# microsoft/M3P

Hardware: AMD Instinct MI355X
Metric: pre-train samples/sec (whole node), 12L/768d seq=128+36 (higher is better)
Workload: dtype bf16; 1 GPU; cfg2: 12L/768d/12h, 36 regions + 128 tokens, V=250002, 19 MLM targets/seq + ITM BCE, dropout 0.10, adam_inverse_sqrt + clip 5; per_gpu_batch=256, global_batch=256, seq_len=164, parallelism=dp1, prewarm_steps=36

## Files before the change

### include/m3p_hip.h

```cpp
#ifndef M3P_HIP_H
#define M3P_HIP_H

#include <stddef.h>
#include <stdint.h>

#ifdef __cplusplus
extern "C" {
#endif

#define M3P_API __attribute__((visibility("default")))

#define M3P_OK 0
#define M3P_EINVAL (-1)
#define M3P_ENOTIMPL (-2)
#define M3P_ENOMEM (-3)

M3P_API const char* m3p_version(void);


enum {
  M3P_EPI_NONE = 0,
  M3P_EPI_BIAS = 1,
  M3P_EPI_BIAS_GELU = 2,
  M3P_EPI_BIAS_DROP_RES = 3,
  M3P_EPI_RES = 4,
  M3P_EPI_DGELU = 5,
  M3P_EPI_MUL = 6,
  M3P_EPI_MULQ = 7,
  M3P_EPI_BIAS_GELUQ = 8,
  M3P_EPI_BIAS_LSE = 9
};

typedef struct M3PEpilogue {
  const float* bias;
  const void* aux;
  void* out2;
  float* colsum;
  int32_t ld_aux;
  int32_t ld_out2;
  int32_t scale_cols;
  float scale;
  float alpha;
  uint32_t seed;
  uint32_t thresh24;
  float inv_keep;
  const float* descale_a;
  const float* descale_b;
  void* out8;
  const float* scale8;
  float* amax8;
  int32_t ld_out8;
  int32_t out8_bf8;
  const int32_t* rng_rows;
  const void* row_ref;
} M3PEpilogue;

M3P_API int m3p_gemm_nt_bf16(const void* A, int lda, const void* W, int ldw, void* C, int ldc,
                             int M, int N, int K, int epilogue, const M3PEpilogue* ep, void* stream);

M3P_API int m3p_gemm_nt_fp8(const void* A8, int lda, int a_is_bf8, const void* W8, int ldw, void* C, int ldc,
                            int M, int N, int K, int epilogue, const M3PEpilogue* ep, void* stream);

M3P_API int m3p_quant_fp8(const void* src, int ld_src, void* dst, int ld_dst, int rows, int cols, const float* scale,
                          float* amax, int bf8, void* stream);

M3P_API int m3p_quant_fp8_batch(const long long* desc, int n_desc, int blocks_per_matrix, void* stream);

M3P_API int m3p_gemm_nt_streamk_f32(const void* A, int lda, const void* W, int ldw, float* C, int ldc,
                                    int M, int N, int K, float alpha, void* stream);
M3P_API int m3p_gemm_nn_streamk_f32(const void* A, int lda, const void* W, int ldw, int k_valid, float* C,
                                    int ldc, int M, int N, int K, float alpha, void* stream);
M3P_API int m3p_gemm_nn_w4_f32(const void* A, int lda, const void* W, int ldw, float* C, int ldc, int M, int N, int K, float alpha,
                               void* workspace, size_t workspace_bytes, void* stream);

M3P_API size_t m3p_gemm_wgrad_workspace_bytes(void);
M3P_API int m3p_gemm_wgrad_bf16(const void* dY, int lddy, const void* X, int ldx, float* dW, int lddw,
                                int M, int N, int K, float alpha, void* workspace, size_t workspace_bytes,
                                void* stream);
M3P_API int m3p_gemm_wgrad_store_bf16(const void* dY, int lddy, const void* X, int ldx, float* dW, int lddw, int M, int N, int K,
                                      float alpha, void* workspace, size_t workspace_bytes, void* stream);
M3P_API int m3p_gemm_wgrad_pair_bf16(const void* dYa, int lddya, const void* Xa, int ldxa, float* dWa, int lddwa, int Na, int Ka,
                                     const void* dYb, int lddyb, const void* Xb, int ldxb, float* dWb, int lddwb, int Nb, int Kb,
                                     int M, float alpha, void* workspace, size_t workspace_bytes, void* stream);


M3P_API int m3p_layernorm_fwd(const void* x, const float* gamma, const float* beta, const uint8_t* rowmask,
                              void* y, float* mean, float* rstd, int rows, int d, float eps, void* stream);

M3P_API int m3p_layernorm_bwd(const void* dy_a, const void* dy_b, const void* x, const float* gamma,
                              const float* mean, const float* rstd, const uint8_t* rowmask,
                              void* dx, void* dx_drop, float* dgamma, float* dbeta, float* dbias_drop,
                              int rows, int d, uint32_t seed, uint32_t thresh24, float inv_keep, void* stream);
M3P_API int m3p_layernorm_bwd_rows(const void* dy_a, const void* dy_b, const void* x, const float* gamma,
                                   const float* mean, const float* rstd, const uint8_t* rowmask,
                                   void* dx, void* dx_drop, float* dgamma, float* dbeta, float* dbias_drop,
                                   int rows, int d, uint32_t seed, uint32_t thresh24, float inv_keep,
                                   const int32_t* rng_rows, void* stream);


M3P_API int m3p_attn_fwd(const void* qkv, const int32_t* keylen, void* ctx, float* lse, uint64_t* keepmask,
                         int B, int S, int H, int dh, uint32_t seed, uint32_t thresh24, float inv_keep,
                         void* stream);

M3P_API int m3p_attn_bwd(const void* qkv, const int32_t* keylen, const void* ctx, const void* dctx,
                         const float* lse, const uint64_t* keepmask, void* dqkv, float* dbias_qkv, int B, int S,
                         int H, int dh, float qscale, uint32_t seed, uint32_t thresh24, float inv_keep,
                         void* stream);

M3P_API int m3p_attn_query_fwd(const void* q, int ld_q, const void* kv, long long kv_bstride, int ld_kv,
                               const int32_t* klen, void* ctx, int B, int Tq, int H, int dh, int Lk, int causal,
                               int pos0, void* stream);

M3P_API int m3p_attn_query_owner_fwd(const void* q, int ld_q, const void* kv, long long kv_bstride, int ld_kv,
                                     const int32_t* klen, void* ctx, int B, int Tq, int H, int dh, int Lk, int causal,
                                     int pos0, const int32_t* owner, int owner_bstride, int owner_kstride, void* stream);

M3P_API int m3p_vocab_select_max_k(void);
M3P_API int m3p_vocab_select_plan(int n, int V, int ld, int beam, int k);
M3P_API size_t m3p_vocab_select_workspace_bytes(int n, int V, int k);
M3P_API int m3p_vocab_select(const void* logits, int ld, int n, int V, const float* beam_scores, int beam, int k,
                             void* workspace, size_t workspace_bytes, float* scores, long long* flat_idx, float* lse,
                             void* stream);

M3P_API int m3p_vocab_sample_plan(int n, int V, int ld, int top_k);
M3P_API size_t m3p_vocab_sample_workspace_bytes(int n, int V, int top_k);
M3P_API int m3p_vocab_sample(const void* logits, int ld, int n, int V, float inv_t, int top_k, uint32_t seed, void* workspace,
                             size_t workspace_bytes, long long* words, float* logprob, float* key, void* stream);

M3P_API int m3p_attn_rows_fwd(const void* q, int ld_q, const void* kv, long long kv_bstride, int ld_kv, const int32_t* klen,
                              void* ctx, float* lse, int B, int Tq, int H, int dh, int Lk, int causal, int pos0,
                              uint32_t seed, uint32_t thresh24, float inv_keep, void* stream);
M3P_API int m3p_attn_rows_bwd(const void* q, int ld_q, const void* kv, long long kv_bstride, int ld_kv, const int32_t* klen,
                              const void* dctx, const float* lse, void* dq, int ld_dq, float* dkv, int B, int Tq, int H,
                              int dh, int Lk, int causal, int pos0, float qscale, uint32_t seed, uint32_t thresh24,
                              float inv_keep, void* stream);

M3P_API int m3p_attn_causal_fwd(const void* qkv, int ld_qkv, void* ctx, float* lse, int B, int T, int H, int dh,
                                uint32_t seed, uint32_t thresh24, float inv_keep, void* stream);
M3P_API int m3p_attn_causal_bwd(const void* qkv, int ld_qkv, const void* dctx, const float* lse, void* dqkv, int ld_dqkv,
                                int B, int T, int H, int dh, float qscale, uint32_t seed, uint32_t thresh24,
                                float inv_keep, void* stream);

M3P_API int m3p_attn_cross_fwd(const void* q, int ld_q, const void* kv, long long kv_bstride, int ld_kv, const int32_t* klen,
                               void* ctx, float* lse, int B, int Tq, int H, int dh, int Lk, uint32_t seed, uint32_t thresh24,
                               float inv_keep, void* stream);
M3P_API int m3p_attn_cross_bwd(const void* q, int ld_q, const void* kv, long long kv_bstride, int ld_kv, const int32_t* klen,
                               const void* dctx, const float* lse, void* dq, int ld_dq, void* dkv, int ld_dkv, int B, int Tq,
                               int H, int dh, int Lk, float qscale, uint32_t seed, uint32_t thresh24, float inv_keep,
                               void* stream);


M3P_API int m3p_cast_f32_bf16(const float* src, void* dst, long long n, void* stream);

M3P_API int m3p_embed_assemble_fwd(const int64_t* tok, const void* emb_bf16, const float* pos,
                                   const void* img_proj, const float* loc, const float* w_loc,
                                   const float* b_loc, const float* g_img, const float* be_img,
                                   const float* g_emb, const float* be_emb, const int32_t* totlen,
                                   void* h, void* z, float* mean_emb, float* rstd_emb, void* e,
                                   float* mean_img, float* rstd_img, int B, int T, int R, int d,
                                   uint32_t seed_img, uint32_t seed_emb, uint32_t thresh24, float inv_keep,
                                   const void* img_rows, void* stream);

M3P_API int m3p_embed_image_rows_fwd(const void* img_proj, const float* loc, const float* w_loc, const float* b_loc,
                                     const float* g_img, const float* be_img, void* e, float* mean_img,
                                     float* rstd_img, void* img_rows, int B, int R, int d, uint32_t seed_img,
                                     uint32_t thresh24, float inv_keep, void* stream);

M3P_API int m3p_embed_assemble_bwd(const void* dh, const void* z, const float* mean_emb, const float* rstd_emb,
                                   const float* g_emb, const void* e, const float* mean_img,
                                   const float* rstd_img, const float* g_img, const int64_t* tok,
                                   const int32_t* totlen, const float* loc, void* dz_scratch, void* de,
                                   float* d_g_emb, float* d_be_emb, float* d_pos, float* d_emb,
                                   void* d_tok_rows, float* d_g_img, float* d_be_img, float* d_b_img, float* d_b_loc,
                                   float* d_w_loc, int B, int T, int R, int d, int pad_index,
                                   uint32_t seed_img, uint32_t seed_emb, uint32_t thresh24, float inv_keep,
                                   int phase, void* stream);


M3P_API int m3p_gather_rows(const void* src, const int32_t* idx, void* dst, int n, int d, void* stream);
M3P_API int m3p_place_rows(const void* src, const int32_t* inv, void* dst, int rows, int d, int n, uint32_t fill_bits,
                           void* stream);
M3P_API int m3p_scatter_add_rows(const void* src, const int32_t* idx, void* dst, int n, int d, void* stream);
M3P_API int m3p_scatter_add_token_rows(const void* rows, int ld_rows, const int64_t* ids, float* dst, int n, int d,
                                       int pad_index, void* stream);

M3P_API int m3p_itm_score_fwd(const void* pre, const float* w2, const float* b2, float* pooled, float* scores, int B,
                              int d, void* stream);
M3P_API int m3p_itm_score_bwd(const float* dscores, const float* pooled, const float* w2, void* dpre16, void* dpreT16,
                              int ldt, float* db1, float* dw2, float* db2, int B, int d, void* stream);

M3P_API int m3p_ce_fwd_bwd(void* logits, int ld, int n_rows, int V, const int64_t* target, float* row_loss,
                           float* loss_sum, float loss_scale, float grad_scale, void* stream);

M3P_API int m3p_ce_lse_from_blocks(const void* stats, int n_blocks, int n_rows, const void* logits, int ld, const int64_t* target,
                                   float* row_loss, float* row_lse, void* scratch, void* stream);
M3P_API int m3p_ce_bwd_colsum(void* logits, int ld, int n_rows, int V, const int64_t* target, const float* row_lse,
                              float grad_scale, float* colsum, void* workspace, size_t workspace_bytes, void* stream);
M3P_API size_t m3p_ce_colsum_workspace_bytes(int ld, int n_rows);
M3P_API int m3p_ce_fwd_bwd_colsum(void* logits, int ld, int n_rows, int V, const int64_t* target, float* row_loss,
                                  float* row_lse, float grad_scale, float* colsum, void* workspace,
                                  size_t workspace_bytes, void* stream);

M3P_API int m3p_ce_shift_target(const void* h, const void* emb, const float* bias, const int64_t* target, float* row_t, void* row_ref,
                                int n_rows, int d, void* stream);
M3P_API int m3p_ce_shift_rows(const void* stats, int n_blocks, int n_rows, float grad_scale, float* row_loss, float* row_s,
                              float* row_q, void* scratch, void* stream);
M3P_API int m3p_ce_shift_colsum(const void* e, int ld, int n_rows, const float* row_s, float* colsum, void* workspace,
                                size_t workspace_bytes, void* stream);
M3P_API int m3p_ce_shift_scale_rows(const void* h, const float* row_s, const float* g, void* out, int n_rows, int d, void* stream);
M3P_API int m3p_ce_shift_target_rows(const void* h, const int64_t* target, const float* row_q, const float* g, float* demb, float* dbias,
                                     int n_rows, int d, void* stream);
M3P_API int m3p_ce_shift_dh(const float* dh32, const void* emb, const int64_t* target, const float* row_s, const float* row_q,
                            const float* g, void* dh, int n_rows, int d, void* stream);

M3P_API int m3p_ce_eval(const void* logits, int ld, int n_rows, int V, const int64_t* target, float* row_loss,
                        int32_t* row_argmax, void* stream);

M3P_API int m3p_colsum_bf16(const void* x, int ld, int n, int ncols, float* out, const float* scale_ptr,
                            void* stream);


M3P_API int m3p_sumsq_f32(const float* g, long long n, double* out, void* stream);

M3P_API int m3p_sumsq_ranges_f32(const float* base, const long long* starts, const long long* counts, int n_ranges, double* out,
                                 void* stream);

M3P_API int m3p_adam_step(float* p, float* g, float* m, float* v, void* w16, long long n, float lr, float beta1,
                          float beta2, float eps, float weight_decay, float step_size, const double* gnorm_sq,
                          float max_norm, float grad_scale, int zero_grad, void* stream);
M3P_API int m3p_adam_step_ranges(float* p, float* g, float* m, float* v, void* w16, const long long* starts,
                                 const long long* counts, const float* step_sizes, const int* zero_grad, int n_ranges,
                                 float lr, float beta1, float beta2, float eps, float weight_decay, const double* gnorm_sq,
                                 float max_norm, float grad_scale, void* stream);

M3P_API int m3p_gelu_fwd(const void* u, void* h, void* dh, long long n, void* stream);
M3P_API int m3p_gelu_fwd_gq(const void* u, void* h, void* gq, int M, int N, void* stream);
M3P_API int m3p_gelu_fwd_q8(const void* u, void* h, void* h8, long long n, const float* scale, float* amax, void* stream);

M3P_API int m3p_gelu_bwd(const void* dy, const void* u, void* du, long long n, void* stream);

M3P_API int m3p_mse_fwd_bwd(const void* pred, int ld_pred, const float* tgt, int ld_tgt, void* dpred, float* row_sq,
                            int rows, int cols, float grad_scale, void* stream);


M3P_API int m3p_dropout_rows(const void* x, int ldx, const void* res, int ldres, void* y, int ldy, int rows, int cols,
                             uint32_t rng_ld, uint32_t rng_col0, uint32_t seed, uint32_t thresh24, float inv_keep,
                             void* stream);

M3P_API int m3p_glu_fwd(const void* ab, int ld_ab, void* y, int rows, int d, void* stream);
M3P_API int m3p_glu_bwd(const void* ab, int ld_ab, const void* dy, void* dab, int rows, int d, void* stream);

M3P_API int m3p_transpose_batch_bf16(const long long* desc, int n_desc, int max_tiles, void* stream);

M3P_API int m3p_transpose_bf16(const void* src, void* dst, int rows, int cols, int ld_src, int ld_dst,
                               void* stream);

M3P_API int m3p_set_persistent_grid(int workgroups);
M3P_API int m3p_set_tile_queue(int32_t* counters, int n_slots);

enum {
  M3P_KERN_NT_SKINNY = 1,
// ... 39 lines not shown
```

### m3p_amd/csrc/attention.hip

```cpp
#include "common.hpp"


namespace {

constexpr int ATTN_BWD_NW = 4;
constexpr int ATTN_BWD_WPS = 3;

static int g_attn_variant = 0;

template <int DH> struct AttnCfg {
  static constexpr int ROWB = DH * 2;
  static constexpr int CH = DH / 8;
  static constexpr int RPI = 1024 / ROWB;
  static constexpr int KK = DH / 32;
  static constexpr int NT = DH / 16;
  static __device__ __forceinline__ int swz(int chunk, int row) { return DH == 64 ? (chunk ^ (row & 7)) : chunk; }
};

__device__ __forceinline__ bf16x4 lds_tr16(const char* p) {
  s16x4 v = __builtin_amdgcn_ds_read_tr16_b64_v4i16((__attribute__((address_space(3))) s16x4*)(p));
  return __builtin_bit_cast(bf16x4, v);
}
__device__ __forceinline__ float row16_sum(float v) {
#define M3P_DPP_ADD(ctrl) v += __builtin_bit_cast(float, __builtin_amdgcn_update_dpp(0, __builtin_bit_cast(int, v), ctrl, 0xf, 0xf, true))
  M3P_DPP_ADD(0xB1);
  M3P_DPP_ADD(0x4E);
  M3P_DPP_ADD(0x124);
  M3P_DPP_ADD(0x128);
#undef M3P_DPP_ADD
  return v;
}
__device__ __forceinline__ uint32_t bit_to_mask(uint32_t bits, int r) {
  uint32_t o;
  switch (r) {
    case 0: asm("v_bfe_i32 %0, %1, 0, 1" : "=v"(o) : "v"(bits)); break;
    case 1: asm("v_bfe_i32 %0, %1, 1, 1" : "=v"(o) : "v"(bits)); break;
    case 2: asm("v_bfe_i32 %0, %1, 2, 1" : "=v"(o) : "v"(bits)); break;
    default: asm("v_bfe_i32 %0, %1, 3, 1" : "=v"(o) : "v"(bits)); break;
  }
  return o;
}
template <int CH>
__device__ __forceinline__ float chunks_sum(float v) {
#define M3P_DPP_ADD(ctrl) v += __builtin_bit_cast(float, __builtin_amdgcn_update_dpp(0, __builtin_bit_cast(int, v), ctrl, 0xf, 0xf, true))
  M3P_DPP_ADD(0xB1);
  M3P_DPP_ADD(0x4E);
  if (CH == 8) M3P_DPP_ADD(0x141);
#undef M3P_DPP_ADD
  return v;
}
__device__ __forceinline__ bf16x8 cat8(bf16x4 a, bf16x4 b) {
  return bf16x8{a[0], a[1], a[2], a[3], b[0], b[1], b[2], b[3]};
}

typedef unsigned int u32x2_t __attribute__((ext_vector_type(2)));
typedef unsigned int u32x4_t __attribute__((ext_vector_type(4)));
template <int NT>
__device__ __forceinline__ void store_row_widened(bf16* row, int fg, bool ok, const bf16x4 (&r)[NT]) {
  static_assert(NT % 2 == 0, "d-tiles are swapped in pairs");
  bf16* p = row + 8 * (fg >> 1) + 16 * (fg & 1);
#pragma unroll
  for (int n0 = 0; n0 < NT; n0 += 2) {
    u32x2_t x = __builtin_bit_cast(u32x2_t, r[n0]), y = __builtin_bit_cast(u32x2_t, r[n0 + 1]);
    asm volatile("s_nop 1\n\tv_permlane16_swap_b32 %0, %2\n\tv_permlane16_swap_b32 %1, %3"
                 : "+v"(x[0]), "+v"(x[1]), "+v"(y[0]), "+v"(y[1]));
    if (ok) *reinterpret_cast<u32x4_t*>(p + 16 * n0) = u32x4_t{x[0], x[1], y[0], y[1]};
  }
}

template <int DH>
__device__ __forceinline__ void stage_rows(const bf16* __restrict__ g, size_t ld, int S, int nrows, char* lds,
                                           int wid, int lane, int nwaves = 4) {
  using Cf = AttnCfg<DH>;
  const int rin = lane / Cf::CH, c = lane % Cf::CH;
  const int ninstr = (nrows + Cf::RPI - 1) / Cf::RPI;
  for (int i = wid; i < ninstr; i += nwaves) {
    const int row = i * Cf::RPI + rin;
    const int gr = min(row, S - 1);
    const int gc = Cf::swz(c, row);
    __builtin_amdgcn_global_load_lds(GLB_PTR(g + (size_t)gr * ld + gc * 8), LDS_PTR(lds + i * 1024), 16, 0, 0);
  }
}

template <int DH>
__device__ __forceinline__ void stage_rows_hidden(const bf16* __restrict__ g, size_t ld, int S, int nrows, char* lds,
                                                  int wid, int lane, int nwaves) {
  using Cf = AttnCfg<DH>;
  const int rin = lane / Cf::CH, c = lane % Cf::CH;
  const int ninstr = (nrows + Cf::RPI - 1) / Cf::RPI;
  const uint32_t lds0 = (uint32_t)(uintptr_t)(__attribute__((address_space(3))) char*)lds;
  for (int i = wid; i < ninstr; i += nwaves) {
    const int row = i * Cf::RPI + rin;
    const int gr = min(row, S - 1);
    const int gc = Cf::swz(c, row);
    const bf16* src = g + (size_t)gr * ld + gc * 8;
    const uint32_t dst = __builtin_amdgcn_readfirstlane(lds0 + (uint32_t)i * 1024u);
    asm volatile("s_mov_b32 m0, %1\n\ts_nop 0\n\tglobal_load_lds_dwordx4 %0, off" :: "v"(src), "s"(dst) : "memory", "m0");
  }
}

template <int DH, int KT, bool DROP, int NTC, int NW = 4, bool EVENS = false>
__global__ __launch_bounds__(NW * 64, NW == 8 ? 2 : 3)
void attn_fwd_kernel(const bf16* __restrict__ qkv, const int* __restrict__ keylen, bf16* __restrict__ ctx,
                     float* __restrict__ lse, unsigned long long* __restrict__ keepmask, int S, int H, int dmodel,
                     uint32_t seed, uint32_t thresh24, float inv_keep) {
  using Cf = AttnCfg<DH>;
  extern __shared__ __attribute__((aligned(16))) char smem[];
  const int tid = threadIdx.x, lane = tid & 63;
  const int wid = __builtin_amdgcn_readfirstlane(tid >> 6);
  const int b = blockIdx.x / H, h = blockIdx.x - b * H;
  const int nt = NTC ? NTC : (S + 15) >> 4;
  const int nk = (nt + 1) >> 1;
  const size_t ld = 3 * (size_t)dmodel;
  const bf16* Qg = qkv + (size_t)b * S * ld + h * DH;
  const bf16* Kg = Qg + dmodel;
  const bf16* Vg = Qg + 2 * dmodel;
  char* sK = smem;
  char* sV = smem + nt * 16 * Cf::ROWB;
  stage_rows<DH>(Kg, ld, S, nt * 16, sK, wid, lane, NW);
  stage_rows<DH>(Vg, ld, S, nk * 32, sV, wid, lane, NW);
  const int fq = lane & 15, fg = lane >> 4;
  const int wrot = (wid + (blockIdx.x >> 3)) & (NW - 1);
  bf16x8 qnext[Cf::KK];
  {
    const int qc0 = min(wrot * 16 + fq, S - 1);
#pragma unroll
    for (int kk = 0; kk < Cf::KK; ++kk)
      qnext[kk] = *reinterpret_cast<const bf16x8*>(Qg + (size_t)qc0 * ld + 32 * kk + 8 * fg);
  }
  const int klen = keylen[b];
  __syncthreads();

  int k_off[Cf::KK];
#pragma unroll
  for (int kk = 0; kk < Cf::KK; ++kk) k_off[kk] = fq * Cf::ROWB + Cf::swz(4 * kk + fg, fq) * 16;
  const int vrow = 4 * fg + (fq >> 2);
  int v_off[Cf::NT];
#pragma unroll
  for (int n = 0; n < Cf::NT; ++n)
    v_off[n] = vrow * Cf::ROWB + Cf::swz(2 * n + ((fq & 3) >> 1), vrow) * 16 + 8 * (fq & 1);

  for (int qb = wrot; qb < nt; qb += NW) {
    const int q = qb * 16 + fq;
    const int qc = min(q, S - 1);
    bf16x8 qf[Cf::KK];
#pragma unroll
    for (int kk = 0; kk < Cf::KK; ++kk) qf[kk] = qnext[kk];
    {
      const int qcn = min(q + 16 * NW, S - 1);
#pragma unroll
      for (int kk = 0; kk < Cf::KK; ++kk)
        qnext[kk] = *reinterpret_cast<const bf16x8*>(Qg + (size_t)qcn * ld + 32 * kk + 8 * fg);
    }

    f32x4 s[2 * KT];
#pragma unroll
    for (int t = 0; t < 2 * KT; ++t) s[t] = f32x4{0.f, 0.f, 0.f, 0.f};
#pragma unroll
    for (int kk = 0; kk < Cf::KK; ++kk) {
#pragma unroll
      for (int t = 0; t < 2 * KT; ++t)
        if (t < nt) {
          const bf16x8 kf = *reinterpret_cast<const bf16x8*>(sK + t * 16 * Cf::ROWB + k_off[kk]);
          s[t] = __builtin_amdgcn_mfma_f32_16x16x32_bf16(kf, qf[kk], s[t], 0, 0, 0);
        }
    }
    constexpr float kLog2e = 1.4426950408889634f;
    float mx = -INFINITY;
    int klen_it = klen;
    asm volatile("" : "+s"(klen_it));
#pragma unroll
    for (int t = 0; t < 2 * KT; ++t)
      if (t < nt) {
        if (16 * t + 16 > klen_it) {
#pragma unroll
          for (int r = 0; r < 4; ++r) s[t][r] = (16 * t + 4 * fg + r < klen_it) ? s[t][r] : -INFINITY;
        }
#pragma unroll
        for (int r = 0; r < 4; ++r) mx = fmaxf(mx, s[t][r]);
      }
    mx = fmaxf(mx, __shfl_xor(mx, 16, 64));
    mx = fmaxf(mx, __shfl_xor(mx, 32, 64));
    const float mx2 = mx * kLog2e;
    float sum = 0.f;
#pragma unroll
    for (int t = 0; t < 2 * KT; ++t)
      if (t < nt) {
#pragma unroll
        for (int r = 0; r < 4; ++r) {
          const float p = __builtin_amdgcn_exp2f(__builtin_fmaf(s[t][r], kLog2e, -mx2));
          s[t][r] = p;
          sum += p;
        }
      }
    sum += __shfl_xor(sum, 16, 64);
    sum += __shfl_xor(sum, 32, 64);
    const float inv = 1.0f / sum;
    const uint32_t rbase = (uint32_t)((b * H + h) * S + qc) * (uint32_t)S;
    const uint32_t thr16 = thresh24 >> 8;
    const bool even_rows = EVENS || (S & 1) == 0;
    unsigned long long* mrow = keepmask ? keepmask + ((size_t)(b * H + h) * nt + qb) * nt * 4 : nullptr;
    constexpr int MW = (8 * KT + 63) / 64;
    uint32_t mlo[MW], mhi[MW];
#pragma unroll
    for (int g = 0; g < MW; ++g) mlo[g] = mhi[g] = 0u;
    bf16x8 pf[KT];
#pragma unroll
    for (int kk = 0; kk < KT; ++kk) {
      float p[8];
      const float invk = DROP ? inv * inv_keep : inv;
      bool kq[8] = {true, true, true, true, true, true, true, true};
      if (DROP) {
#pragma unroll
        for (int hf = 0; hf < 2; ++hf) {
          const int t = 2 * kk + hf;
          if (t < nt) {
            const uint32_t base = rbase + (uint32_t)(16 * t + 4 * fg);
            bool k4[4];
            if (even_rows) {
              asm volatile("" ::: "memory");
              const uint32_t h0 = m3p_hash32(base >> 1, seed), h1 = m3p_hash32((base >> 1) + 1u, seed);
              k4[0] = (h0 & 0xFFFFu) >= thr16; k4[1] = (h0 >> 16) >= thr16;
              k4[2] = (h1 & 0xFFFFu) >= thr16; k4[3] = (h1 >> 16) >= thr16;
            } else {
              asm volatile("" ::: "memory");
              m3p_keep_run<4>(base, seed, thresh24, k4);
            }
#pragma unroll
            for (int r = 0; r < 4; ++r) kq[4 * hf + r] = k4[r];
          }
        }
      }
#pragma unroll
      for (int hf = 0; hf < 2; ++hf) {
        const int t = 2 * kk + hf;
        unsigned long long kw[4] = {0ull, 0ull, 0ull, 0ull};
#pragma unroll
        for (int r = 0; r < 4; ++r) {
          const int j = 4 * hf + r;
          float v = 0.f;
          if (t < nt) {
            v = s[t][r] * invk;
            if (DROP) {
              const bool keep = kq[j];
              kw[r] = __builtin_amdgcn_ballot_w64(keep);
              v = keep ? v : 0.f;
            }
          }
          p[j] = v;
        }
        if (DROP && t < nt) {
          asm("s_nop 3\n\tv_writelane_b32 %0, %2, %10\n\tv_writelane_b32 %1, %3, %10\n\tv_writelane_b32 %0, %4, %11\n\tv_writelane_b32 %1, %5, %11\n\t"
              "v_writelane_b32 %0, %6, %12\n\tv_writelane_b32 %1, %7, %12\n\tv_writelane_b32 %0, %8, %13\n\tv_writelane_b32 %1, %9, %13"
              : "+v"(mlo[(4 * t) >> 6]), "+v"(mhi[(4 * t) >> 6])
              : "s"((uint32_t)kw[0]), "s"((uint32_t)(kw[0] >> 32)), "s"((uint32_t)kw[1]), "s"((uint32_t)(kw[1] >> 32)),
                "s"((uint32_t)kw[2]), "s"((uint32_t)(kw[2] >> 32)), "s"((uint32_t)kw[3]), "s"((uint32_t)(kw[3] >> 32)),
                "i"((4 * t) & 63), "i"((4 * t + 1) & 63), "i"((4 * t + 2) & 63), "i"((4 * t + 3) & 63));
        }
      }
      pf[kk] = bf16x8{(bf16)p[0], (bf16)p[1], (bf16)p[2], (bf16)p[3], (bf16)p[4], (bf16)p[5], (bf16)p[6], (bf16)p[7]};
    }
    if (DROP && mrow) {
#pragma unroll
      for (int g = 0; g < MW; ++g)
        if (64 * g + lane < 4 * nt) mrow[64 * g + lane] = ((unsigned long long)mhi[g] << 32) | mlo[g];
    }
    f32x4 o[Cf::NT];
#pragma unroll
    for (int n = 0; n < Cf::NT; ++n) o[n] = f32x4{0.f, 0.f, 0.f, 0.f};
#pragma unroll
    for (int kk = 0; kk < KT; ++kk) {
      if (kk < nk) {
#pragma unroll
        for (int n = 0; n < Cf::NT; ++n) {
          const char* pv = sV + kk * 32 * Cf::ROWB + v_off[n];
          const bf16x8 vf = cat8(lds_tr16(pv), lds_tr16(pv + 16 * Cf::ROWB));
          o[n] = __builtin_amdgcn_mfma_f32_16x16x32_bf16(vf, pf[kk], o[n], 0, 0, 0);
        }
      }
    }
    {
      bf16x4 ob[Cf::NT];
#pragma unroll
      for (int n = 0; n < Cf::NT; ++n) ob[n] = bf16x4{(bf16)o[n][0], (bf16)o[n][1], (bf16)o[n][2], (bf16)o[n][3]};
      store_row_widened<Cf::NT>(ctx + (size_t)(b * S + min(q, S - 1)) * dmodel + h * DH, fg, q < S, ob);
      if (q < S && fg == 0) lse[(size_t)(b * H + h) * S + q] = mx + __logf(sum);
    }
  }
}

template <int DH, int KT, bool DROP, bool MASK, int NKC, int NTC, int NW = 4, int KB = 1, int KBQ = KB, bool ONEPASS = false>
__global__ __launch_bounds__(NW * 64, NTC == 11 ? ATTN_BWD_WPS : ((NW == 8 || KB == 2) ? 2 : 3))
void attn_bwd_kernel(const bf16* __restrict__ qkv, const int* __restrict__ keylen, const bf16* __restrict__ ctx,
                     const bf16* __restrict__ dctx, const float* __restrict__ lse,
                     const unsigned long long* __restrict__ keepmask, bf16* __restrict__ dqkv,
                     float* __restrict__ dbias_qkv, int S, int H, int dmodel, float qscale, uint32_t seed,
                     uint32_t thresh24, float inv_keep) {
  using Cf = AttnCfg<DH>;
  extern __shared__ __attribute__((aligned(16))) char smem[];
  const int tid = threadIdx.x, lane = tid & 63;
  const int wid = __builtin_amdgcn_readfirstlane(tid >> 6);
  const int b = blockIdx.x / H, h = blockIdx.x - b * H;
  const int wrot = (NW & (NW - 1)) ? wid : ((wid + (blockIdx.x >> 3)) & (NW - 1));
  const int nt = NTC ? NTC : ((S + 15) >> 4);
  const int nk = NKC ? NKC : ((S + 31) >> 5);
  const size_t ld = 3 * (size_t)dmodel;
  const int b_rd = b;
  const bf16* Qg = qkv + (size_t)b_rd * S * ld + h * DH;
  const bf16* Kg = Qg + dmodel;
  const bf16* Vg = Qg + 2 * dmodel;
  const bf16* Og = ctx + (size_t)b_rd * S * dmodel + h * DH;
  const bf16* dOg = dctx + (size_t)b_rd * S * dmodel + h * DH;
  bf16* dQg = dqkv + (size_t)b * S * ld + h * DH;
  bf16* dKg = dQg + dmodel;
  bf16* dVg = dQg + 2 * dmodel;
  const float* lse_bh = lse + (size_t)(b * H + h) * S;
  const int klen = keylen[b];
  const unsigned long long* mbh = MASK ? keepmask + (size_t)(b * H + h) * nt * nt * 4 : nullptr;

  const int tile_bytes = nk * 32 * Cf::ROWB;
  char* s0 = smem;
  char* s1 = smem + tile_bytes;
  float* sL = reinterpret_cast<float*>(smem + 2 * tile_bytes);
  float* sD = sL + nk * 32;
  const int fq = lane & 15, fg = lane >> 4;
  float* sB = sD + nk * 32;
  float* sBw = sB + wid * 3 * DH;
  constexpr int DSP = NTC * 32;
  char* sK = reinterpret_cast<char*>(sB + NW * 3 * DH);
  char* sDS = sK + tile_bytes;
  static_assert(!ONEPASS || (NKC == 6 && NTC == 11 && KB == 1 && DH == 64), "ONEPASS is the M3P-sequence instantiation");
  f32x4 bsum[Cf::NT];
#pragma unroll
  for (int n = 0; n < Cf::NT; ++n) bsum[n] = f32x4{0.f, 0.f, 0.f, 0.f};
  auto bias_acc = [&](int, int n, const bf16x4& v4) {
    bsum[n] += f32x4{(float)v4[0], (float)v4[1], (float)v4[2], (float)v4[3]};
  };
  auto bias_flush = [&](int part) {
#pragma unroll
    for (int n = 0; n < Cf::NT; ++n) {
      f32x4 x = bsum[n];
#pragma unroll
      for (int r = 0; r < 4; ++r) x[r] = row16_sum(x[r]);
      if (fq == 0) *reinterpret_cast<f32x4*>(sBw + part * DH + 16 * n + 4 * fg) = x;
      bsum[n] = f32x4{0.f, 0.f, 0.f, 0.f};
    }
  };

  int r_off[Cf::KK];
#pragma unroll
  for (int kk = 0; kk < Cf::KK; ++kk) r_off[kk] = fq * Cf::ROWB + Cf::swz(4 * kk + fg, fq) * 16;
  const int trow = 4 * fg + (fq >> 2);
  int t_off[Cf::NT];
#pragma unroll
  for (int n = 0; n < Cf::NT; ++n)
    t_off[n] = trow * Cf::ROWB + Cf::swz(2 * n + ((fq & 3) >> 1), trow) * 16 + 8 * (fq & 1);

#define PAD_TILE(t) (NTC ? (t) >= NTC : (!MASK && (t) >= nt))
  constexpr float kLog2e = 1.4426950408889634f;
  constexpr float kMasked = -1.0e30f;
  constexpr bool kDfromLds = NKC != 0;
  constexpr int kStageInstr = NKC * 32 / Cf::RPI;
  constexpr int kNIW = kDfromLds ? (kStageInstr + NW - 1) / NW : 1;
  bf16x8 orow[kNIW];
  if (kDfromLds) {
    const int rin = lane / Cf::CH, c = lane % Cf::CH;
#pragma unroll
    for (int j = 0; j < kNIW; ++j) {
      const int row = (wid + j * NW) * Cf::RPI + rin;
      orow[j] = *reinterpret_cast<const bf16x8*>(Og + (size_t)min(row, S - 1) * dmodel + Cf::swz(c, row) * 8);
    }
  }
  stage_rows<DH>(Qg, ld, S, nk * 32, s0, wid, lane, NW);
  stage_rows<DH>(dOg, (size_t)dmodel, S, nk * 32, s1, wid, lane, NW);
  if (ONEPASS) stage_rows<DH>(Kg, ld, S, nk * 32, sK, wid, lane, NW);
  bf16x8 kf[KB][Cf::KK], vf[KB][Cf::KK];
  auto load_kv = [&](int u, int kb) {
    const int keyc = min(kb * 16 + fq, S - 1);
#pragma unroll
    for (int kk = 0; kk < Cf::KK; ++kk) {
      kf[u][kk] = *reinterpret_cast<const bf16x8*>(Kg + (size_t)keyc * ld + 32 * kk + 8 * fg);
      vf[u][kk] = *reinterpret_cast<const bf16x8*>(Vg + (size_t)keyc * ld + 32 * kk + 8 * fg);
    }
  };
  constexpr bool kNextFrag = NKC != 0 && NTC != 0 && !(DROP && !MASK);
  bf16x8 kfn[KB][Cf::KK], vfn[KB][Cf::KK];
  auto load_kv_next = [&](int u, int kb) {
    const int keyc = min(kb * 16 + fq, S - 1);
#pragma unroll
    for (int kk = 0; kk < Cf::KK; ++kk) {
      kfn[u][kk] = *reinterpret_cast<const bf16x8*>(Kg + (size_t)keyc * ld + 32 * kk + 8 * fg);
      vfn[u][kk] = *reinterpret_cast<const bf16x8*>(Vg + (size_t)keyc * ld + 32 * kk + 8 * fg);
    }
  };
  if (wrot * KB < nt) {
#pragma unroll
    for (int u = 0; u < KB; ++u) load_kv(u, wrot * KB + u);
  }
  const float log2_inv_keep = DROP ? __builtin_amdgcn_logf(inv_keep) : 0.f;
  const float keep_prob = DROP ? __builtin_amdgcn_rcpf(inv_keep) : 1.f;
  for (int q = tid; q < nk * 32; q += NW * 64) {
    float dsum = 0.f, l = INFINITY;
    if (q < S) {
      if (!kDfromLds) {
        const bf16* op = Og + (size_t)q * dmodel;
        const bf16* dp = dOg + (size_t)q * dmodel;
#pragma unroll
        for (int c = 0; c < DH / 8; ++c) {
          const bf16x8 ov = *reinterpret_cast<const bf16x8*>(op + 8 * c);
          const bf16x8 dv = *reinterpret_cast<const bf16x8*>(dp + 8 * c);
#pragma unroll
          for (int e = 0; e < 8; ++e) dsum += (float)ov[e] * (float)dv[e];
        }
      }
      l = lse_bh[q] * kLog2e - log2_inv_keep;
    }
    if (!kDfromLds) sD[q] = dsum * keep_prob;
    sL[q] = l;
  }
  if (kDfromLds) {
    asm volatile("s_waitcnt vmcnt(0)" ::: "memory");
    const int rin = lane / Cf::CH, c = lane % Cf::CH;
#pragma unroll
    for (int j = 0; j < kNIW; ++j) {
      const int i = wid + j * NW;
      if (i < kStageInstr) {
        const bf16x8 dv = *reinterpret_cast<const bf16x8*>(s1 + i * 1024 + lane * 16);
        float part = 0.f;
#pragma unroll
        for (int e = 0; e < 8; ++e) part += (float)orow[j][e] * (float)dv[e];
        part = chunks_sum<Cf::CH>(part);
        const int row = i * Cf::RPI + rin;
        if (c == 0) sD[row] = row < S ? part * keep_prob : 0.f;
      }
    }
  }
  __syncthreads();

  constexpr bool kPreA = MASK && NKC != 0;
// ... 209 lines not shown
  }
  __syncthreads();

  for (int qb0 = wrot * KBQ; qb0 < nt; qb0 += NW * KBQ) {
    int q[KBQ], qc[KBQ];
    float lq[KBQ], dq_[KBQ];
    uint32_t rbase[KBQ];
#pragma unroll
    for (int u = 0; u < KBQ; ++u) {
      q[u] = (qb0 + u) * 16 + fq;
      qc[u] = min(q[u], S - 1);
      if (kNextFrag) {
        if (qb0 != wrot * KBQ) {
#pragma unroll
          for (int kk = 0; kk < Cf::KK; ++kk) { qf[u][kk] = qfn[u][kk]; df[u][kk] = dfn[u][kk]; }
        }
        if (qb0 + NW * KBQ < nt) load_qd_next(u, qb0 + NW * KBQ + u);
      } else if (qb0 != wrot * KBQ) {
        load_qd(u, qb0 + u);
      }
      const bool in = q[u] < nk * 32;
      lq[u] = in ? sL[min(q[u], nk * 32 - 1)] : INFINITY;
      dq_[u] = in ? sD[min(q[u], nk * 32 - 1)] : 0.f;
      rbase[u] = (uint32_t)((b * H + h) * S + qc[u]) * (uint32_t)S;
    }
    int klen_it = klen;
    asm volatile("" : "+s"(klen_it));
    constexpr bool kPreB = MASK && NKC != 0;
    unsigned long long mwB[2][KBQ][2][4];
    auto mask_words_B = [&](int kq_, int par) {
#pragma unroll
      for (int u = 0; u < KBQ; ++u)
#pragma unroll
        for (int hf = 0; hf < 2; ++hf) {
          const unsigned long long* mw_ = mbh + ((size_t)min(qb0 + u, nt - 1) * nt + min(2 * kq_ + hf, nt - 1)) * 4;
#pragma unroll
          for (int r = 0; r < 4; ++r) mwB[par][u][hf][r] = mw_[r];
        }
    };
    if (kPreB) mask_words_B(0, 0);
    f32x4 dq[KBQ][Cf::NT];
#pragma unroll
    for (int u = 0; u < KBQ; ++u)
#pragma unroll
      for (int n = 0; n < Cf::NT; ++n) dq[u][n] = f32x4{0.f, 0.f, 0.f, 0.f};
#pragma unroll(NKC ? NKC : 1)
    for (int kq = 0; kq < nk; ++kq) {
      if (kPreB && kq + 1 < nk) mask_words_B(kq + 1, (kq + 1) & 1);
      f32x4 scB[KBQ][2], dpB[KBQ][2];
#pragma unroll
      for (int u = 0; u < KBQ; ++u)
#pragma unroll
        for (int hf = 0; hf < 2; ++hf) {
          scB[u][hf] = f32x4{0.f, 0.f, 0.f, 0.f};
          dpB[u][hf] = DROP ? f32x4{0.f, 0.f, 0.f, 0.f} : f32x4{-dq_[u], -dq_[u], -dq_[u], -dq_[u]};
        }
#pragma unroll
      for (int kk = 0; kk < Cf::KK; ++kk) {
#pragma unroll
        for (int hf = 0; hf < 2; ++hf) {
          const int t = 2 * kq + hf;
          if (PAD_TILE(t)) continue;
          const bf16x8 kfr = *reinterpret_cast<const bf16x8*>(s0 + t * 16 * Cf::ROWB + r_off[kk]);
          const bf16x8 vfr = *reinterpret_cast<const bf16x8*>(s1 + t * 16 * Cf::ROWB + r_off[kk]);
#pragma unroll
          for (int u = 0; u < KBQ; ++u) {
            scB[u][hf] = __builtin_amdgcn_mfma_f32_16x16x32_bf16(kfr, qf[u][kk], scB[u][hf], 0, 0, 0);
            dpB[u][hf] = __builtin_amdgcn_mfma_f32_16x16x32_bf16(vfr, df[u][kk], dpB[u][hf], 0, 0, 0);
          }
        }
      }
      bf16x8 sfrag[KBQ];
#pragma unroll
      for (int u = 0; u < KBQ; ++u) {
        f32x4 ds2[2];
#pragma unroll
        for (int hf = 0; hf < 2; ++hf) {
          const int t = 2 * kq + hf;
          if (PAD_TILE(t)) {
            ds2[hf] = f32x4{0.f, 0.f, 0.f, 0.f};
            continue;
          }
          f32x4 sc = scB[u][hf];
          const f32x4 dp = dpB[u][hf];
          const unsigned long long* mw = MASK ? mbh + ((size_t)min(qb0 + u, nt - 1) * nt + min(t, nt - 1)) * 4 : nullptr;
          if (16 * t + 16 > klen_it) {
            asm volatile("");
#pragma unroll
            for (int r = 0; r < 4; ++r) sc[r] = (16 * t + 4 * fg + r < klen_it) ? sc[r] : kMasked;
          }
#pragma unroll
          for (int r = 0; r < 4; ++r) {
            const int key = 16 * t + 4 * fg + r;
            const float p = __builtin_amdgcn_exp2f(__builtin_fmaf(sc[r], kLog2e, -lq[u]));
            if (DROP) {
              float kfac;
              if (MASK) {
                asm("v_cndmask_b32_e64 %0, 0, 1.0, %1" : "=v"(kfac) : "s"(kPreB ? mwB[kq & 1][u][hf][r] : mw[r]));
              } else {
                static_assert(MASK || !DROP, "dropout in backward reads the forward pass's keep words");
                kfac = 1.f;
              }
              ds2[hf][r] = p * __builtin_fmaf(dp[r], kfac, -dq_[u]);
            } else {
              ds2[hf][r] = p * dp[r];
            }
          }
        }
        sfrag[u] = bf16x8{(bf16)ds2[0][0], (bf16)ds2[0][1], (bf16)ds2[0][2], (bf16)ds2[0][3],
                          (bf16)ds2[1][0], (bf16)ds2[1][1], (bf16)ds2[1][2], (bf16)ds2[1][3]};
      }
#pragma unroll
      for (int n = 0; n < Cf::NT; ++n) {
        const char* pk = s0 + kq * 32 * Cf::ROWB + t_off[n];
        const bf16x8 kT = cat8(lds_tr16(pk), lds_tr16(pk + 16 * Cf::ROWB));
#pragma unroll
        for (int u = 0; u < KBQ; ++u) dq[u][n] = __builtin_amdgcn_mfma_f32_16x16x32_bf16(kT, sfrag[u], dq[u][n], 0, 0, 0);
      }
      if (NKC) __builtin_amdgcn_sched_barrier(0);
    }
#pragma unroll
    for (int u = 0; u < KBQ; ++u) {
      bf16x4 qb4[Cf::NT];
#pragma unroll
      for (int n = 0; n < Cf::NT; ++n)
        qb4[n] = bf16x4{(bf16)(dq[u][n][0] * qscale), (bf16)(dq[u][n][1] * qscale), (bf16)(dq[u][n][2] * qscale), (bf16)(dq[u][n][3] * qscale)};
      const bool ok = q[u] < S;
      if (dbias_qkv) {
#pragma unroll
        for (int n = 0; n < Cf::NT; ++n) bias_acc(0, n, ok ? qb4[n] : bf16x4{0, 0, 0, 0});
      }
      store_row_widened<Cf::NT>(dQg + (size_t)qc[u] * ld, fg, ok, qb4);
    }
  }
  }

  if (dbias_qkv) {
    bias_flush(0);
    __syncthreads();
    for (int i = tid; i < 3 * DH; i += NW * 64) {
      const int part = i / DH, c = i - part * DH;
      if (part != 1) {
        float tot = 0.f;
#pragma unroll
        for (int w = 0; w < NW; ++w) tot += sB[w * 3 * DH + i];
        atomicAdd(dbias_qkv + part * dmodel + h * DH + c, tot);
      }
    }
  }
}

#undef PAD_TILE

template <bool DROP, bool MASK>
__global__ __launch_bounds__(768, 3)
void attn_bwd_p_kernel(const bf16* __restrict__ qkv, const int* __restrict__ keylen, const bf16* __restrict__ ctx,
                       const bf16* __restrict__ dctx, const float* __restrict__ lse,
                       const unsigned long long* __restrict__ keepmask, bf16* __restrict__ dqkv,
                       float* __restrict__ dbias_qkv, int S, int H, int dmodel, int nheads, float qscale, float inv_keep) {
  constexpr int DH = 64, NW = 12, NKC = 6, NTC = 11, NR = NKC * 32;
  using Cf = AttnCfg<DH>;
  constexpr int DSP = NTC * 32;
  constexpr int TILE = NR * Cf::ROWB;
  extern __shared__ __attribute__((aligned(16))) char smem[];
  const int tid = threadIdx.x, lane = tid & 63;
  const int wid = __builtin_amdgcn_readfirstlane(tid >> 6);
  char* s0 = smem;
  char* s1 = s0 + TILE;
  char* sK = s1 + TILE;
  char* sDS = sK + TILE;
  float* sL = reinterpret_cast<float*>(sDS + NTC * 16 * DSP);
  float* sD = sL + NR;
  float* sB = sD + NR;
  unsigned long long* sMW = reinterpret_cast<unsigned long long*>(sB + 2 * NW * 3 * DH) + wid * 48;
  const size_t ld = 3 * (size_t)dmodel;
  const int fq = lane & 15, fg = lane >> 4;
  const int rin = lane / Cf::CH, c8 = lane % Cf::CH;
  int r_off[Cf::KK];
#pragma unroll
  for (int kk = 0; kk < Cf::KK; ++kk) r_off[kk] = fq * Cf::ROWB + Cf::swz(4 * kk + fg, fq) * 16;
  const int trow = 4 * fg + (fq >> 2);
  int t_off[Cf::NT];
#pragma unroll
  for (int n = 0; n < Cf::NT; ++n)
    t_off[n] = trow * Cf::ROWB + Cf::swz(2 * n + ((fq & 3) >> 1), trow) * 16 + 8 * (fq & 1);
  constexpr float kLog2e = 1.4426950408889634f;
  constexpr float kMasked = -1.0e30f;
  const float log2_inv_keep = DROP ? __builtin_amdgcn_logf(inv_keep) : 0.f;
  const float keep_prob = DROP ? __builtin_amdgcn_rcpf(inv_keep) : 1.f;
  constexpr int kStageInstr = NR / Cf::RPI;
  constexpr int kNIW = (kStageInstr + NW - 1) / NW;
#define PAD_TILE(t) ((t) >= NTC)

  bf16x8 orow[kNIW], kf[Cf::KK], vf[Cf::KK];
  float lse_r = 0.f;
  unsigned long long mw_req = 0;
  auto request_head = [&](int hd) {
    const int b = hd / H, h = hd - b * H;
    const bf16* Qg = qkv + (size_t)b * S * ld + h * DH;
    const bf16* Og = ctx + (size_t)b * S * dmodel + h * DH;
    const bf16* dOg = dctx + (size_t)b * S * dmodel + h * DH;
#pragma unroll
    for (int j = 0; j < kNIW; ++j) {
      const int row = (wid + j * NW) * Cf::RPI + rin;
      orow[j] = *reinterpret_cast<const bf16x8*>(Og + (size_t)min(row, S - 1) * dmodel + Cf::swz(c8, row) * 8);
    }
    stage_rows_hidden<DH>(Qg, ld, S, NR, s0, wid, lane, NW);
    stage_rows_hidden<DH>(dOg, (size_t)dmodel, S, NR, s1, wid, lane, NW);
    const int keyc = min(min(wid, NTC - 1) * 16 + fq, S - 1);
#pragma unroll
    for (int kk = 0; kk < Cf::KK; ++kk) {
      kf[kk] = *reinterpret_cast<const bf16x8*>(Qg + dmodel + (size_t)keyc * ld + 32 * kk + 8 * fg);
      vf[kk] = *reinterpret_cast<const bf16x8*>(Qg + 2 * dmodel + (size_t)keyc * ld + 32 * kk + 8 * fg);
    }
    if (tid < NR && tid < S) lse_r = lse[(size_t)hd * S + tid];
    if (MASK && lane < 4 * NTC)
      mw_req = keepmask[(size_t)hd * NTC * NTC * 4 + ((size_t)(lane >> 2) * NTC + min(wid, NTC - 1)) * 4 + (lane & 3)];
  };

  f32x4 bsum[Cf::NT];
#pragma unroll
  for (int n = 0; n < Cf::NT; ++n) bsum[n] = f32x4{0.f, 0.f, 0.f, 0.f};
  auto bias_acc = [&](int n, const bf16x4& v4) { bsum[n] += f32x4{(float)v4[0], (float)v4[1], (float)v4[2], (float)v4[3]}; };
  auto bias_flush = [&](float* slot, int part) {
    float t[2][4], u[4];
#pragma unroll
    for (int n = 0; n < 2; ++n)
#pragma unroll
      for (int r = 0; r < 4; ++r) {
        asm volatile("v_add_f32_dpp %0, %1, %1 row_ror:8 row_mask:0xf bank_mask:0x3" : "=v"(t[n][r]) : "v"(bsum[n][r]));
        asm volatile("v_add_f32_dpp %0, %1, %1 row_ror:8 row_mask:0xf bank_mask:0xc" : "+v"(t[n][r]) : "v"(bsum[n + 2][r]));
      }
    asm volatile("s_nop 1");
#pragma unroll
    for (int r = 0; r < 4; ++r) {
      asm volatile("v_add_f32_dpp %0, %1, %1 row_half_mirror row_mask:0xf bank_mask:0x5" : "=v"(u[r]) : "v"(t[0][r]));
      asm volatile("v_add_f32_dpp %0, %1, %1 row_half_mirror row_mask:0xf bank_mask:0xa" : "+v"(u[r]) : "v"(t[1][r]));
    }
    asm volatile("s_nop 1");
    f32x4 x;
#pragma unroll
    for (int r = 0; r < 4; ++r) {
      float v = u[r];
      v += __builtin_bit_cast(float, __builtin_amdgcn_update_dpp(0, __builtin_bit_cast(int, v), 0xB1, 0xf, 0xf, true));
      v += __builtin_bit_cast(float, __builtin_amdgcn_update_dpp(0, __builtin_bit_cast(int, v), 0x4E, 0xf, 0xf, true));
      x[r] = v;
    }
    if ((fq & 3) == 0) *reinterpret_cast<f32x4*>(slot + part * DH + 16 * (fq >> 2) + 4 * fg) = x;
#pragma unroll
    for (int n = 0; n < Cf::NT; ++n) bsum[n] = f32x4{0.f, 0.f, 0.f, 0.f};
  };
  auto bias_reduce = [&](const float* slots, int h) {
    for (int i = tid; i < 3 * DH; i += NW * 64) {
      const int part = i / DH, c = i - part * DH;
      if (part != 1) {
        float tot = 0.f;
#pragma unroll
        for (int w = 0; w < NW; ++w) tot += slots[w * 3 * DH + i];
        atomicAdd(dbias_qkv + part * dmodel + h * DH + c, tot);
      }
    }
  };

  bf16x4 kb4[Cf::NT], vb4[Cf::NT], qb4[Cf::NT];
  const int key = wid * 16 + fq;
  bf16* dQg_prev = nullptr;
  auto store_head = [&](bf16* dQh) {
    if (wid < NTC) {
      bf16* row = dQh + (size_t)min(key, S - 1) * ld;
      store_row_widened<Cf::NT>(row, fg, key < S, qb4);
      store_row_widened<Cf::NT>(row + dmodel, fg, key < S, kb4);
      store_row_widened<Cf::NT>(row + 2 * dmodel, fg, key < S, vb4);
    }
  };
  int hd = blockIdx.x;
  if (hd >= nheads) return;
  constexpr int kStagger = 2;
  for (int i = 0; i < (int)((blockIdx.x >> 3) & 3) * kStagger; ++i) __builtin_amdgcn_s_sleep(16);
  request_head(hd);
  int par = 0, prev_h = -1;
  for (;;) {
    const int b = hd / H, h = hd - b * H;
    bf16* dQg = dqkv + (size_t)b * S * ld + h * DH;
    const bf16* Kg = qkv + (size_t)b * S * ld + h * DH + dmodel;
    const int klen = keylen[b];
    float* sBh = sB + par * (NW * 3 * DH);
    __builtin_amdgcn_s_waitcnt(0x0F70);
    asm volatile("s_waitcnt vmcnt(0)" ::: "memory");
#pragma unroll
    for (int j = 0; j < kNIW; ++j) {
      const int i = wid + j * NW;
      if (i < kStageInstr) {
        const bf16x8 dvv = *reinterpret_cast<const bf16x8*>(s1 + i * 1024 + lane * 16);
        float part = 0.f;
#pragma unroll
        for (int e = 0; e < 8; ++e) part += (float)orow[j][e] * (float)dvv[e];
        part = chunks_sum<Cf::CH>(part);
        const int row = i * Cf::RPI + rin;
        if (c8 == 0) sD[row] = row < S ? part * keep_prob : 0.f;
      }
    }
    if (tid < NR) sL[tid] = tid < S ? lse_r * kLog2e - log2_inv_keep : INFINITY;
    if (MASK && lane < 4 * NTC) sMW[lane] = mw_req;
    asm volatile("s_waitcnt lgkmcnt(0)" ::: "memory");
    __builtin_amdgcn_s_barrier();
    asm volatile("" ::: "memory");
    if (prev_h >= 0 && dbias_qkv) bias_reduce(sB + (par ^ 1) * (NW * 3 * DH), prev_h);
    if (prev_h >= 0) store_head(dQg_prev);
    dQg_prev = dQg;
    stage_rows_hidden<DH>(Kg, ld, S, NR, sK, wid, lane, NW);
    if (wid < NTC) {
      const float kbias = (key < klen) ? 0.f : kMasked;
      f32x4 dv[Cf::NT], dk[Cf::NT];
#pragma unroll
      for (int n = 0; n < Cf::NT; ++n) dv[n] = dk[n] = f32x4{0.f, 0.f, 0.f, 0.f};
#pragma unroll
      for (int kq = 0; kq < NKC; ++kq) {
        f32x4 scA[2], dpA[2], dnegA[2];
#pragma unroll
        for (int hf = 0; hf < 2; ++hf) {
          const int t = 2 * kq + hf;
          dnegA[hf] = f32x4{-sD[16 * t + 4 * fg + 0], -sD[16 * t + 4 * fg + 1], -sD[16 * t + 4 * fg + 2], -sD[16 * t + 4 * fg + 3]};
          scA[hf] = f32x4{kbias, kbias, kbias, kbias};
          dpA[hf] = DROP ? f32x4{0.f, 0.f, 0.f, 0.f} : dnegA[hf];
        }
#pragma unroll
        for (int kk = 0; kk < Cf::KK; ++kk) {
#pragma unroll
          for (int hf = 0; hf < 2; ++hf) {
            const int t = 2 * kq + hf;
            if (PAD_TILE(t)) continue;
            const bf16x8 qf = *reinterpret_cast<const bf16x8*>(s0 + t * 16 * Cf::ROWB + r_off[kk]);
            const bf16x8 df = *reinterpret_cast<const bf16x8*>(s1 + t * 16 * Cf::ROWB + r_off[kk]);
            scA[hf] = __builtin_amdgcn_mfma_f32_16x16x32_bf16(qf, kf[kk], scA[hf], 0, 0, 0);
            dpA[hf] = __builtin_amdgcn_mfma_f32_16x16x32_bf16(df, vf[kk], dpA[hf], 0, 0, 0);
          }
        }
        f32x4 pd2[2], ds2[2];
#pragma unroll
        for (int hf = 0; hf < 2; ++hf) {
          const int t = 2 * kq + hf;
          if (PAD_TILE(t)) {
            pd2[hf] = ds2[hf] = f32x4{0.f, 0.f, 0.f, 0.f};
            continue;
          }
          uint32_t kbits = 0;
          if (MASK) kbits = (uint32_t)(sMW[4 * t + (fq & 3)] >> (4 * fg + 16 * (fq >> 2)));
#pragma unroll
          for (int r = 0; r < 4; ++r) {
            const int q = 16 * t + 4 * fg + r;
            const float p = __builtin_amdgcn_exp2f(__builtin_fmaf(scA[hf][r], kLog2e, -sL[q]));
            if (DROP) {
              const float pd = __builtin_bit_cast(float, __builtin_bit_cast(uint32_t, p) & bit_to_mask(kbits, r));
              pd2[hf][r] = pd;
              ds2[hf][r] = __builtin_fmaf(pd, dpA[hf][r], p * dnegA[hf][r]);
            } else {
              pd2[hf][r] = p;
              ds2[hf][r] = p * dpA[hf][r];
            }
          }
        }
        const bf16x8 pfrag = bf16x8{(bf16)pd2[0][0], (bf16)pd2[0][1], (bf16)pd2[0][2], (bf16)pd2[0][3],
                                    (bf16)pd2[1][0], (bf16)pd2[1][1], (bf16)pd2[1][2], (bf16)pd2[1][3]};
        const bf16x8 sfrag = bf16x8{(bf16)ds2[0][0], (bf16)ds2[0][1], (bf16)ds2[0][2], (bf16)ds2[0][3],
                                    (bf16)ds2[1][0], (bf16)ds2[1][1], (bf16)ds2[1][2], (bf16)ds2[1][3]};
#pragma unroll
        for (int hf = 0; hf < 2; ++hf) {
          if (PAD_TILE(2 * kq + hf)) continue;
          *reinterpret_cast<bf16x4*>(sDS + key * DSP + (32 * kq + 16 * hf + 4 * fg) * 2) =
              hf ? bf16x4{sfrag[4], sfrag[5], sfrag[6], sfrag[7]} : bf16x4{sfrag[0], sfrag[1], sfrag[2], sfrag[3]};
        }
#pragma unroll
        for (int n = 0; n < Cf::NT; ++n) {
          const char* pq = s0 + kq * 32 * Cf::ROWB + t_off[n];
          const char* pdo = s1 + kq * 32 * Cf::ROWB + t_off[n];
          const bf16x8 qT = cat8(lds_tr16(pq), lds_tr16(pq + 16 * Cf::ROWB));
          const bf16x8 dT = cat8(lds_tr16(pdo), lds_tr16(pdo + 16 * Cf::ROWB));
          dv[n] = __builtin_amdgcn_mfma_f32_16x16x32_bf16(dT, pfrag, dv[n], 0, 0, 0);
          dk[n] = __builtin_amdgcn_mfma_f32_16x16x32_bf16(qT, sfrag, dk[n], 0, 0, 0);
        }
        __builtin_amdgcn_sched_barrier(0);
      }
#pragma unroll
      for (int n = 0; n < Cf::NT; ++n) {
        kb4[n] = bf16x4{(bf16)dk[n][0], (bf16)dk[n][1], (bf16)dk[n][2], (bf16)dk[n][3]};
        vb4[n] = bf16x4{(bf16)dv[n][0], (bf16)dv[n][1], (bf16)dv[n][2], (bf16)dv[n][3]};
        if (dbias_qkv) bias_acc(n, key < S ? vb4[n] : bf16x4{0, 0, 0, 0});
      }
    }
    if (dbias_qkv) bias_flush(sBh + wid * 3 * DH, 2);
    __builtin_amdgcn_s_waitcnt(0);
    asm volatile("s_waitcnt vmcnt(0) lgkmcnt(0)" ::: "memory");
    __builtin_amdgcn_s_barrier();
    asm volatile("" ::: "memory");
    const int next = hd + gridDim.x;
    if (next < nheads) request_head(next);
    if (wid < NTC) {
      f32x4 dq[Cf::NT];
#pragma unroll
      for (int n = 0; n < Cf::NT; ++n) dq[n] = f32x4{0.f, 0.f, 0.f, 0.f};
      const char* pds = sDS + trow * DSP + wid * 32 + (fq & 3) * 8;
#pragma unroll
      for (int kq = 0; kq < NKC; ++kq) {
        const bf16x4 lo = lds_tr16(pds + (32 * kq) * DSP);
        const bf16x4 hi = PAD_TILE(2 * kq + 1) ? bf16x4{0, 0, 0, 0} : lds_tr16(pds + (32 * kq + 16) * DSP);
        const bf16x8 sfr = cat8(lo, hi);
#pragma unroll
        for (int n = 0; n < Cf::NT; ++n) {
          const char* pk = sK + kq * 32 * Cf::ROWB + t_off[n];
          const bf16x8 kT = cat8(lds_tr16(pk), lds_tr16(pk + 16 * Cf::ROWB));
          dq[n] = __builtin_amdgcn_mfma_f32_16x16x32_bf16(kT, sfr, dq[n], 0, 0, 0);
        }
      }
#pragma unroll
      for (int n = 0; n < Cf::NT; ++n) {
        qb4[n] = bf16x4{(bf16)(dq[n][0] * qscale), (bf16)(dq[n][1] * qscale), (bf16)(dq[n][2] * qscale), (bf16)(dq[n][3] * qscale)};
        if (dbias_qkv) bias_acc(n, key < S ? qb4[n] : bf16x4{0, 0, 0, 0});
      }
    }
    if (dbias_qkv) bias_flush(sBh + wid * 3 * DH, 0);
    prev_h = h;
    par ^= 1;
    if (next >= nheads) break;
    hd = next;
  }
  store_head(dQg_prev);
  if (dbias_qkv) {
    __syncthreads();
    bias_reduce(sB + (par ^ 1) * (NW * 3 * DH), prev_h);
  }
#undef PAD_TILE
}

template <int DH>
int launch_fwd(const bf16* qkv, const int* keylen, bf16* ctx, float* lse, unsigned long long* keepmask, int B, int S, int H,
               int dmodel, uint32_t seed, uint32_t thresh24, float inv_keep, hipStream_t st) {
  const int nt = (S + 15) / 16, nk = (S + 31) / 32;
  const size_t lds = (size_t)(nt * 16 + nk * 32) * DH * 2;
  const bool wide = 2 * lds > 160 * 1024;
#define M3P_ATTN_FWD(KT)                                                                                        \
  do {                                                                                                          \
    constexpr int NW0 = (KT == 16) ? 8 : 4;    \
    auto kern = thresh24 ? attn_fwd_kernel<DH, KT, true, 0, NW0> : attn_fwd_kernel<DH, KT, false, 0, NW0>;       \
    if (nt == 11 && KT == 6) kern = thresh24 ? ((S & 1) ? attn_fwd_kernel<DH, 6, true, 11> : attn_fwd_kernel<DH, 6, true, 11, 4, true>) \
                                             : attn_fwd_kernel<DH, 6, false, 11>; \
    if (wide) kern = thresh24 ? attn_fwd_kernel<DH, KT, true, 0, 8> : attn_fwd_kernel<DH, KT, false, 0, 8>;       \
    hipError_t e = hipFuncSetAttribute((const void*)kern, hipFuncAttributeMaxDynamicSharedMemorySize, (int)lds); \
    if (e != hipSuccess) return (int)e;                                                                         \
    hipLaunchKernelGGL(kern, dim3(B* H), dim3((wide || NW0 == 8) ? 512 : 256), lds, st, qkv, keylen, ctx, lse, keepmask, S, H, dmodel, seed, \
                       thresh24, inv_keep);                                                                     \
  } while (0)
  if (nk <= 6) M3P_ATTN_FWD(6);
  else if (nk <= 12) M3P_ATTN_FWD(12);
  else if (nk <= 16) M3P_ATTN_FWD(16);
  else return M3P_EINVAL;
#undef M3P_ATTN_FWD
  M3P_CHECK_LAUNCH();
  return M3P_OK;
}

template <int DH>
int launch_bwd(const bf16* qkv, const int* keylen, const bf16* ctx, const bf16* dctx, const float* lse,
               const unsigned long long* keepmask, bf16* dqkv, float* dbias, int B, int S, int H, int dmodel, float qscale,
               uint32_t seed, uint32_t thresh24, float inv_keep, hipStream_t st) {
  const int nk = (S + 31) / 32;
  const bool wide = (size_t)2 * ((size_t)2 * nk * 32 * DH * 2) > 160 * 1024;
  const bool m3p_seq = nk == 6 && (S + 15) / 16 == 11;
  const bool onepass = m3p_seq && DH == 64 && (!thresh24 || keepmask) && !(g_attn_variant & 1);
  const int nwaves = wide ? 8 : (onepass ? 12 : (m3p_seq ? ATTN_BWD_NW : 4));
  const size_t lds = (size_t)2 * nk * 32 * DH * 2 + (size_t)2 * nk * 32 * sizeof(float) + 3 * nwaves * DH * sizeof(float) +
                     (onepass ? (size_t)nk * 32 * DH * 2 + (size_t)11 * 16 * 11 * 32 : 0);
#define M3P_ATTN_BWD(KT, DROP, MASK)                                                                            \
  do {                                                                                                          \
    auto kern = attn_bwd_kernel<DH, KT, DROP, MASK, 0, 0>;                                                      \
    if (wide) kern = attn_bwd_kernel<DH, KT, DROP, MASK, 0, 0, 8>;                                              \
    if (nk == 6) kern = attn_bwd_kernel<DH, KT, DROP, MASK, 6, 0>;                                              \
    if (m3p_seq) kern = attn_bwd_kernel<DH, KT, DROP, MASK, 6, 11, ATTN_BWD_NW, 1, 1>;                                \
    if constexpr (DH == 64 && (MASK || !DROP)) { if (onepass) kern = attn_bwd_kernel<DH, KT, DROP, MASK, 6, 11, 12, 1, 1, true>; } \
    hipError_t e = hipFuncSetAttribute((const void*)kern, hipFuncAttributeMaxDynamicSharedMemorySize, (int)lds); \
    if (e != hipSuccess) return (int)e;                                                                         \
    hipLaunchKernelGGL(kern, dim3(B* H), dim3(nwaves * 64), lds, st, qkv, keylen, ctx, dctx, lse, keepmask, dqkv, dbias, S, H, \
                       dmodel, qscale, seed, thresh24, inv_keep);                                               \
  } while (0)
  if (nk > 16) return M3P_EINVAL;
  if constexpr (DH == 64) {
    if (onepass && !(g_attn_variant & 2)) {
      int dev = 0, n_cu = 0;
      if (hipGetDevice(&dev) != hipSuccess || hipDeviceGetAttribute(&n_cu, hipDeviceAttributeMultiprocessorCount, dev) != hipSuccess || n_cu <= 0)
        n_cu = 256;
      const size_t ldsp = (size_t)3 * 192 * 128 + (size_t)11 * 16 * 11 * 32 + 2 * 192 * sizeof(float) + 2 * 12 * 3 * 64 * sizeof(float) + 12 * 48 * 8;
      auto kp = thresh24 ? attn_bwd_p_kernel<true, true> : attn_bwd_p_kernel<false, false>;
      if (hipFuncSetAttribute((const void*)kp, hipFuncAttributeMaxDynamicSharedMemorySize, (int)ldsp) == hipSuccess) {
        const int nheads = B * H;
        hipLaunchKernelGGL(kp, dim3(nheads < n_cu ? nheads : n_cu), dim3(768), ldsp, st, qkv, keylen, ctx, dctx, lse, keepmask, dqkv, dbias,
                           S, H, dmodel, nheads, qscale, inv_keep);
        M3P_CHECK_LAUNCH();
        return M3P_OK;
      }
      (void)hipGetLastError();
    }
  }
  if (!thresh24) M3P_ATTN_BWD(16, false, false);
  else M3P_ATTN_BWD(16, true, true);
#undef M3P_ATTN_BWD
  M3P_CHECK_LAUNCH();
  return M3P_OK;
}

}

extern "C" {

void m3p_debug_attn_variant(int v) { g_attn_variant = v; }

int m3p_attn_fwd(const void* qkv, const int32_t* keylen, void* ctx, float* lse, uint64_t* keepmask, int B, int S, int H, int dh,
                 uint32_t seed, uint32_t thresh24, float inv_keep, void* stream) {
  if (B <= 0 || S <= 0 || H <= 0 || S > 512) return M3P_EINVAL;
  if (((uintptr_t)qkv & 15) || ((uintptr_t)ctx & 7)) return M3P_EINVAL;
  const int dmodel = H * dh;
  hipStream_t st = (hipStream_t)stream;
  if (dh == 64) return launch_fwd<64>((const bf16*)qkv, keylen, (bf16*)ctx, lse, (unsigned long long*)keepmask, B, S, H, dmodel, seed, thresh24, inv_keep, st);
  if (dh == 32) return launch_fwd<32>((const bf16*)qkv, keylen, (bf16*)ctx, lse, (unsigned long long*)keepmask, B, S, H, dmodel, seed, thresh24, inv_keep, st);
  return M3P_EINVAL;
}

int m3p_attn_bwd(const void* qkv, const int32_t* keylen, const void* ctx, const void* dctx, const float* lse,
                 const uint64_t* keepmask, void* dqkv, float* dbias_qkv, int B, int S, int H, int dh, float qscale,
                 uint32_t seed, uint32_t thresh24, float inv_keep, void* stream) {
  if (B <= 0 || S <= 0 || H <= 0 || S > 512) return M3P_EINVAL;
  if (thresh24 && !keepmask) return M3P_EINVAL;
  if (((uintptr_t)qkv & 15) || ((uintptr_t)ctx & 15) || ((uintptr_t)dctx & 15) || ((uintptr_t)dqkv & 7)) return M3P_EINVAL;
  const int dmodel = H * dh;
  hipStream_t st = (hipStream_t)stream;
  if (dh == 64)
    return launch_bwd<64>((const bf16*)qkv, keylen, (const bf16*)ctx, (const bf16*)dctx, lse, (const unsigned long long*)keepmask, (bf16*)dqkv, dbias_qkv, B, S, H,
                          dmodel, qscale, seed, thresh24, inv_keep, st);
  if (dh == 32)
    return launch_bwd<32>((const bf16*)qkv, keylen, (const bf16*)ctx, (const bf16*)dctx, lse, (const unsigned long long*)keepmask, (bf16*)dqkv, dbias_qkv, B, S, H,
                          dmodel, qscale, seed, thresh24, inv_keep, st);
  return M3P_EINVAL;
}

}
```

### m3p_amd/functional.py

```python
import math
import os
from collections import OrderedDict

import torch

from . import lib as L
from . import fp8 as fp8mod
from . import ops
from . import rng

BF16 = torch.bfloat16
ALIGN = 64
BUCKET_ALIGN = 64 * 8


def _round_up(n, a):
    return (n + a - 1) // a * a


_VOCAB_FULL_TILES = os.environ.get('M3P_VOCAB_FULL_TILES', '1') != '0'
_GELU_GRAD_IN_FWD = os.environ.get('M3P_GELU_GRAD_IN_FWD', '0') != '0'
_GELU_BYTE_GRAD = int(os.environ.get('M3P_GELU_BYTE_GRAD', '2'))
_CE_FUSED_LSE = os.environ.get('M3P_CE_FUSED_LSE', '1') != '0'
_VOCAB_DGRAD_W4 = os.environ.get('M3P_VOCAB_DGRAD_W4', '1') != '0'
# ... 257 lines not shown
        self.out = [ar.w('encoder_attn.%d.out_lin.weight' % i) for i in range(n)]
        self.bq = [ar.xattn(i, 'bq') for i in range(n)]
        self.bkv = [ar.xattn(i, 'bkv') for i in range(n)]
        self.bo = [ar.p('encoder_attn.%d.out_lin.bias' % i) for i in range(n)]


_REF_SITE0 = 1 << 20


def _transposed(w):
    wt = torch.empty((w.shape[1], w.shape[0]), dtype=BF16, device=w.device)
    ops.transpose_bf16(w, wt)
    return wt


def refiner_fwd(model, x, keylen, B, R, seed_step, p):
    ar = model.arena()
    d, H = model.dim, model.n_heads
    dh = d // H
    M = B * R
    qscale = 1.0 / math.sqrt(dh)
    seed = lambda i, k: rng.stream_seed(model.base_seed, seed_step, _REF_SITE0 + 8 * i + k)
    layers = []
    for i in range(model.n_refine_layers):
        pre = 'refine_embeddings.layers.%d.' % i
        xn, mean_a, rstd_a = ops.layernorm_fwd(x, ar.p(pre + 'sublayer.0.norm.weight'), ar.p(pre + 'sublayer.0.norm.bias'))
        qkv = ops.gemm_nt(xn, ar.ref_qkv_w16(i), L.EPI_BIAS, bias=ar.ref_qkv_bias(i), scale_cols=d, scale=qscale)
        ctxt, lse, kmask = ops.attn_fwd(qkv, keylen, B, R, H, dh, seed=seed(i, 0), p_drop=p, want_mask=True)
        cat = torch.empty((M, 2 * d), dtype=BF16, device=x.device)
        ops.dropout_rows(ctxt, p, seed(i, 1), out=cat[:, :d], rng_ld=2 * d, rng_col0=0)
        ops.dropout_rows(xn, p, seed(i, 1), out=cat[:, d:], rng_ld=2 * d, rng_col0=d)
        ab = ops.gemm_nt(cat, ar.w(pre + 'self_attn.aoa_layer.0.weight'), L.EPI_BIAS,
                         bias=ar.p(pre + 'self_attn.aoa_layer.0.bias'))
        x1 = ops.dropout_rows(ops.glu_fwd(ab), p, seed(i, 2), res=x)
        xn2, mean_b, rstd_b = ops.layernorm_fwd(x1, ar.p(pre + 'sublayer.1.norm.weight'), ar.p(pre + 'sublayer.1.norm.bias'))
        u = torch.empty((M, 4 * d), dtype=BF16, device=x.device)
        hact = ops.gemm_nt(xn2, ar.w(pre + 'feed_forward.lin1.weight'), L.EPI_BIAS_GELU,
                           bias=ar.p(pre + 'feed_forward.lin1.bias'), out2=u)
        t = ops.gemm_nt(hact, ar.w(pre + 'feed_forward.lin2.weight'), L.EPI_BIAS, bias=ar.p(pre + 'feed_forward.lin2.bias'))
        if p > 0:
            ops.dropout_rows(t, p, seed(i, 3), out=t)
        x2 = ops.dropout_rows(t, p, seed(i, 4), res=x1)
        layers.append((x, mean_a, rstd_a, xn, qkv, ctxt, lse, kmask, cat, ab, x1, mean_b, rstd_b, xn2, u, hact))
        x = x2
    out, mean_f, rstd_f = ops.layernorm_fwd(x, ar.p('refine_embeddings.norm.weight'), ar.p('refine_embeddings.norm.bias'))
    return out, (layers, x, mean_f, rstd_f)


def refiner_bwd(model, dout, saved, keylen, B, R, seed_step, p):
    ar = model.arena()
    d, H = model.dim, model.n_heads
    dh = d // H
    seed = lambda i, k: rng.stream_seed(model.base_seed, seed_step, _REF_SITE0 + 8 * i + k)
    layers, x_last, mean_f, rstd_f = saved
    dx, _ = ops.layernorm_bwd(dout, None, x_last, ar.p('refine_embeddings.norm.weight'), mean_f, rstd_f, None,
                              ar.g('refine_embeddings.norm.weight'), ar.g('refine_embeddings.norm.bias'))
    for i in reversed(range(model.n_refine_layers)):
        pre = 'refine_embeddings.layers.%d.' % i
        (x, mean_a, rstd_a, xn, qkv, ctxt, lse, kmask, cat, ab, x1, mean_b, rstd_b, xn2, u, hact) = layers[i]
        layers[i] = None
        dt = ops.dropout_rows(dx, p, seed(i, 4))
        if p > 0:
            ops.dropout_rows(dt, p, seed(i, 3), out=dt)
        ops.colsum(dt, d, ar.g(pre + 'feed_forward.lin2.bias'))
        ops.gemm_wgrad(dt, hact, ar.g(pre + 'feed_forward.lin2.weight'))
        du = ops.gemm_nt(dt, _transposed(ar.w(pre + 'feed_forward.lin2.weight')), L.EPI_DGELU, aux=u,
                         colsum=ar.g(pre + 'feed_forward.lin1.bias'))
        ops.gemm_wgrad(du, xn2, ar.g(pre + 'feed_forward.lin1.weight'))
        dxn2 = ops.gemm_nt(du, _transposed(ar.w(pre + 'feed_forward.lin1.weight')), L.EPI_NONE)
        dln, _ = ops.layernorm_bwd(dxn2, None, x1, ar.p(pre + 'sublayer.1.norm.weight'), mean_b, rstd_b, None,
                                   ar.g(pre + 'sublayer.1.norm.weight'), ar.g(pre + 'sublayer.1.norm.bias'))
        dx1 = ops.dropout_rows(dln, 0.0, 0, res=dx)
        del dt, du, dxn2, dln, u, hact, xn2
        dy = ops.dropout_rows(dx1, p, seed(i, 2))
        dab = ops.glu_bwd(ab, dy)
        ops.colsum(dab, 2 * d, ar.g(pre + 'self_attn.aoa_layer.0.bias'))
        ops.gemm_wgrad(dab, cat, ar.g(pre + 'self_attn.aoa_layer.0.weight'))
        dcat = ops.gemm_nt(dab, _transposed(ar.w(pre + 'self_attn.aoa_layer.0.weight')), L.EPI_NONE)
        dctx = ops.dropout_rows(dcat[:, :d], p, seed(i, 1), rng_ld=2 * d, rng_col0=0)
        dxn_cat = ops.dropout_rows(dcat[:, d:], p, seed(i, 1), rng_ld=2 * d, rng_col0=d)
        dqkv = ops.attn_bwd(qkv, keylen, ctxt, dctx, lse, B, R, H, dh, dbias_qkv=ar.ref_qkv_bias(i, grad=True),
                            seed=seed(i, 0), p_drop=p, keepmask=kmask)
        ops.gemm_wgrad(dqkv, xn, ar.ref_qkv_wgrad(i))
        dxn = ops.gemm_nt(dqkv, _transposed(ar.ref_qkv_w16(i)), L.EPI_RES, aux=dxn_cat)
        dln, _ = ops.layernorm_bwd(dxn, None, x, ar.p(pre + 'sublayer.0.norm.weight'), mean_a, rstd_a, None,
                                   ar.g(pre + 'sublayer.0.norm.weight'), ar.g(pre + 'sublayer.0.norm.bias'))
        dx = ops.dropout_rows(dln, 0.0, 0, res=dx1)
        del dy, dab, dcat, dctx, dxn_cat, dqkv, dxn, dln, dx1
    ar.touch(*[n for n in ar.names if n.startswith('refine_embeddings.')])
    return dx


class GradSink:

    def __init__(self):
        self.buf = None

    def rows(self, like):
        if self.buf is None:
            self.buf = torch.zeros_like(like)
        assert self.buf.shape == like.shape
        return self.buf

    def take(self):
        buf, self.buf = self.buf, None
        return buf


def _sink_of(tensor, base):
    root = tensor._base if tensor._is_view() else tensor
    sink = getattr(root, '_m3p_sink', None) if root is not None else None
    if sink is None or base is None or not torch.is_grad_enabled():
        return None
    if root.dim() != 2 or not root.is_contiguous() or root.storage_offset() != 0 or tuple(root.shape) != tuple(base.shape):
        return None
    return sink


def first_rows_sink(model, tensor):
    d = model.dim
    if tensor.dim() != 3 or tensor.dtype != BF16 or not tensor._is_view():
        return None, None, None
    st, soff = tensor.stride(), tensor.storage_offset()
    if st[2] != 1 or st[0] % d or soff % d:
        return None, None, None
    with torch.no_grad():
        base = torch.as_strided(tensor, (tensor.untyped_storage().nbytes() // 2 // d, d), (d, 1), 0)
    sink = _sink_of(tensor, base)
    if sink is None:
        return None, None, None
    cache = model.__dict__.setdefault('_first_rows_cache', {})
    key = (tensor.shape[0], st[0], soff, tensor.device)
    rows = cache.get(key)
    if rows is None:
        rows = ((soff + torch.arange(tensor.shape[0], device=tensor.device, dtype=torch.int64) * st[0]) // d).to(torch.int32)
        cache.clear()
        cache[key] = rows
    return sink, base, rows


N_ENC_ARGS = 17

ROW_TILE = 256
COMPACT_MIN_ROWS = 4096


def compact_rows_eligible(n_rows, M):
    if n_rows <= 0:
        return 0
    n = _round_up(n_rows, ROW_TILE)
    return n if (n >= COMPACT_MIN_ROWS and 2 * n <= M) else 0


class OutputRows:

    def __init__(self, flags):
        flags = torch.as_tensor(flags).reshape(-1).cpu()
        if flags.dtype != torch.bool:
            flags = flags != 0
        self.flags = flags
        self.M = int(flags.numel())
        sel = torch.nonzero(flags).view(-1)
        self.n_rows = int(sel.numel())
        self.n = compact_rows_eligible(self.n_rows, self.M)
        self.idx = self.idx64 = self.inv = None
        if self.n:
            pad = torch.nonzero(~flags).view(-1)[:self.n - self.n_rows]
            idx = torch.cat([sel, pad]).to(torch.int32)
            inv = torch.full((self.M,), -1, dtype=torch.int32)
            inv[sel] = torch.arange(self.n_rows, dtype=torch.int32)
            self._host = (idx, inv)

    @classmethod
    def from_masks(cls, B, S, R, first=True, pred_mask=None, region_labels=None):
        flags = torch.zeros((B, S), dtype=torch.bool)
        if first:
            flags[:, 0] = True
        if pred_mask is not None:
            flags[:, R:] |= torch.as_tensor(pred_mask).cpu().reshape(S - R, B).t() != 0
        if region_labels is not None and R > 0:
            flags[:, :R] |= torch.as_tensor(region_labels).cpu().reshape(B, R) != -1
        return cls(flags)

    def to(self, device):
        if self.n and self.idx is None:
            from .utils import to_cuda
            with torch.cuda.device(device):
                self.idx, self.inv = to_cuda(*self._host)
            self.idx64 = self.idx.long()
        assert self.idx is None or self.idx.device == torch.device(device), 'an OutputRows serves one pass on one device'
        return self


class EncoderFn(torch.autograd.Function):

    @staticmethod
    def forward(ctx, anchor, model, x, lengths, x_img, lengths_img, image_loc, p_drop, p_attn, seed_step, p_refine=None,
                track=False, text_embed=None, langs=None, h0=None, positions=None, out_rows=None):
        ar = model.arena()
        ready = model.ddp_hook.params_ready if model.ddp_hook is not None else (lambda key: None)
        ar.refresh(wait_params=False)
        ready('vocab')
        ready('embed')
        dev = ar.device
        d, H, nL = model.dim, model.n_heads, model.n_layers
        dh = d // H
        seed = lambda kind, i=0: rng.stream_seed(model.base_seed, seed_step, _site(kind, i))
        if h0 is not None:
            assert x is None and x_img is None and text_embed is None and langs is None and positions is None
            B = lengths.shape[0]
            S = h0.shape[0] // B
            T, R, M = S, 0, B * S
            totlen, rowmask = ops.seq_masks(lengths.to(device=dev, dtype=torch.int64).contiguous(), None, B, S)
            h = h0.detach().to(BF16).contiguous()
            ximg16 = loc = emb_saved = img_rows = img_saved = ref_saved = keylen_img = tok = None
        else:
            h = None
            T, B = x.shape
            R = 0 if x_img is None else x_img.shape[0]
            S = R + T
            M = B * S
            x = x.to(dev).contiguous()
        if h is None:
            table, tok = ar.w('embeddings.weight'), x
            if text_embed is not None:
                assert tuple(text_embed.shape) == (B, T, d), (tuple(text_embed.shape), (B, T, d))
                table = text_embed.detach().to(device=dev, dtype=BF16).contiguous().view(B * T, d)
                tok = (torch.arange(B, device=dev, dtype=torch.int64) * T)[None, :] + \
                    torch.arange(T, device=dev, dtype=torch.int64)[:, None]
                tok = tok.contiguous()
            if langs is not None or positions is not None:
                assert text_embed is None and R == 0
                rows = table[x.t()].float()
                if langs is not None:
                    langs = langs.to(dev).contiguous()
                    rows = rows + ar.p('cross_lang_embeddings.weight')[langs.t()]
                if positions is not None:
                    positions = positions.to(dev).contiguous()
                    assert positions.size() == (T, B)
                    ptab = ar.p('position_embeddings.weight')
                    rows = rows + ptab[positions.t()] - ptab[:T][None, :, :]
                table = rows.to(BF16).reshape(B * T, d).contiguous()
                tok = ((torch.arange(B, device=dev, dtype=torch.int64) * T)[None, :] +
                       torch.arange(T, device=dev, dtype=torch.int64)[:, None]).contiguous()
            totlen, rowmask = ops.seq_masks(lengths.to(device=dev, dtype=torch.int64).contiguous(),
                                            None if R == 0 else lengths_img.to(device=dev, dtype=torch.int64).contiguous(), B, S)

            ximg16 = img_proj = loc = None
            if R > 0:
                xi = x_img.detach().to(dev)
                if xi.dtype == torch.float32 and xi.stride(2) == 1 and xi.stride(0) % 4 == 0 and xi.stride(1) % 4 == 0:
                    ximg16 = ops.cast_rows_bf16(xi)
                else:
                    ximg16 = ops.cast_bf16(xi.contiguous().view(R * B, 2048))
                loc = image_loc.contiguous().float()
                img_proj = ops.gemm_nt(ximg16, ar.w('image_embeddings.image_embeddings.weight'), L.EPI_BIAS,
                                       bias=ar.p('image_embeddings.image_embeddings.bias'))
            img_rows = img_saved = ref_saved = keylen_img = None
            if p_refine is not None and R > 0:
                rows, img_saved = ops.embed_image_rows_fwd(
                    img_proj, loc, ar.p('image_embeddings.image_location_embeddings.weight'),
                    ar.p('image_embeddings.image_location_embeddings.bias'), ar.p('image_embeddings.LayerNorm.weight'),
                    ar.p('image_embeddings.LayerNorm.bias'), B, R, d, seed_img=seed('img'), p_drop=p_drop)
                keylen_img = lengths_img.to(device=dev, dtype=torch.int32).contiguous()
                img_rows, ref_saved = refiner_fwd(model, rows, keylen_img, B, R, seed_step, p_refine)
            h, emb_saved = ops.embed_assemble_fwd(
                tok, table, ar.p('position_embeddings.weight'), img_proj, loc,
                ar.p('image_embeddings.image_location_embeddings.weight'),
                ar.p('image_embeddings.image_location_embeddings.bias'),
                ar.p('image_embeddings.LayerNorm.weight'), ar.p('image_embeddings.LayerNorm.bias'),
                ar.p('layer_norm_emb.weight'), ar.p('layer_norm_emb.bias'), totlen, B, T, R, d,
                seed_img=seed('img'), seed_emb=seed('emb'), p_drop=p_drop, img_rows=img_rows, img_saved=img_saved)

        saved_layers = []
        qscale = 1.0 / math.sqrt(dh)
        st8 = model.fp8_state() if model.fp8 else None
        if st8 is not None:
            assert M % 256 == 0, 'the fp8 GEMM takes whole 256-row tiles (B * S %% 256 == 0): M = %d' % M
            if model.training:
                st8.roll()
            ready(None)
            st8.quant_weights(ar)

        def lin(xin, i, xsite, wsite, w16, epi, pre8=None, **kw):
            if st8 is None or wsite not in fp8mod.FWD_SITES:
                return ops.gemm_nt(xin, w16, epi, **kw)
            x8, dxs = pre8 if pre8 is not None else st8.quant(xin, i, xsite)
            w8, _, dws = st8.weights[(i, wsite)]
            return ops.gemm_nt_fp8(x8, w8, epi, descale_a=dxs, descale_b=dws, **kw)

        rows_c = None
        if out_rows is not None and out_rows.n and track and st8 is None and nL > 0 and d % 8 == 0 \
                and ops.gq_eligible(M, 4 * d) == ops.gq_eligible(out_rows.n, 4 * d):
            assert out_rows.M == M, 'out_rows was built for %d rows, this pass has %d' % (out_rows.M, M)
            rows_c = out_rows.to(dev)

        for i in range(nL):
            a, f = 'attentions.%d.' % i, 'ffns.%d.' % i
            ready(('layer', i))
            qkv = lin(h, i, 'x', 'wqkv', ar.qkv_w16(i), L.EPI_BIAS, bias=ar.qkv_bias(i), scale_cols=d, scale=qscale)
            ctxt, lse, kmask = ops.attn_fwd(qkv, totlen, B, S, H, dh, seed=seed('attn_p', i), p_drop=p_attn,
                                            want_mask=True)
            lse = (lse, kmask)
            compact = rows_c is not None and i == nL - 1
            Mi, ctx_in, res_in, mask_i, rr, ctx_c = M, ctxt, h, rowmask, {}, None
            if compact:
                Mi, rr = rows_c.n, dict(rng_rows=rows_c.idx)
                ctx_in = ctx_c = ops.gather_rows(ctxt, rows_c.idx, Mi, d)
                res_in = ops.gather_rows(h, rows_c.idx, Mi, d)
                mask_i = rowmask[rows_c.idx64]
            pre1 = lin(ctx_in, i, 'ctx', 'wout', ar.w(a + 'out_lin.weight'), L.EPI_BIAS_DROP_RES, bias=ar.p(a + 'out_lin.bias'),
                       aux=res_in, seed=seed('attn_out', i), p_drop=p_drop, **rr)
            x1, mean1, rstd1 = ops.layernorm_fwd(pre1, ar.p('layer_norm1.%d.weight' % i), ar.p('layer_norm1.%d.bias' % i))
            hact8 = None
            u_holds_grad = False
            if (st8 is None or 'w1' not in fp8mod.FWD_SITES) and not _GELU_GRAD_IN_FWD and _GELU_BYTE_GRAD == 2 and track \
                    and ops.gq_eligible(Mi, 4 * d):
                u = torch.empty((Mi * 4 * d,), dtype=torch.uint8, device=dev)
                o8 = {}
                if st8 is not None and 'w2' in fp8mod.FWD_SITES:
                    kh = st8.index(i, 'hact')
                    if st8.seen[kh]:
                        o8 = dict(out8=torch.empty((M, 4 * d), dtype=torch.uint8, device=dev), scale8=st8.scale[kh:kh + 1],
                                  amax8=st8.amax[kh:kh + 1])
                hact = ops.gemm_nt(x1, ar.w(f + 'lin1.weight'), L.EPI_BIAS_GELUQ, bias=ar.p(f + 'lin1.bias'), out2=u, **o8)
                if o8:
                    hact8 = (o8['out8'], st8.descale[kh:kh + 1])
                elif st8 is not None and 'w2' in fp8mod.FWD_SITES:
                    st8._first_use(hact, kh)
                u_holds_grad = 'q'
            elif Mi >= 1024 or st8 is not None:
                u = lin(x1, i, 'x1', 'w1', ar.w(f + 'lin1.weight'), L.EPI_BIAS, bias=ar.p(f + 'lin1.bias'))
                if st8 is not None and 'w2' in fp8mod.FWD_SITES and 'w2' not in fp8mod.BWD_SITES and not _GELU_GRAD_IN_FWD:
                    hact, hact8 = st8.gelu_quant(u, i)
                elif st8 is None and not _GELU_GRAD_IN_FWD and _GELU_BYTE_GRAD and track and ops.gq_eligible(Mi, 4 * d):
                    hact, u = ops.gelu_fwd_gq(u)
                    u_holds_grad = 'q'
                else:
                    u_holds_grad = _GELU_GRAD_IN_FWD or (st8 is not None and 'w2' in fp8mod.BWD_SITES)
                    hact = ops.gelu_fwd(u, grad_inplace=u_holds_grad)
            else:
                u = torch.empty((Mi, 4 * d), dtype=BF16, device=dev)
                hact = ops.gemm_nt(x1, ar.w(f + 'lin1.weight'), L.EPI_BIAS_GELU, bias=ar.p(f + 'lin1.bias'), out2=u)
            pre2 = lin(hact, i, 'hact', 'w2', ar.w(f + 'lin2.weight'), L.EPI_BIAS_DROP_RES, bias=ar.p(f + 'lin2.bias'),
                       aux=x1, seed=seed('ffn', i), p_drop=p_drop, pre8=hact8, **rr)
            h_next, mean2, rstd2 = ops.layernorm_fwd(pre2, ar.p('layer_norm2.%d.weight' % i),
                                                     ar.p('layer_norm2.%d.bias' % i), mask_i)
            if track:
                saved_layers.append((h, qkv, ctxt, lse, pre1, mean1, rstd1, x1, u, hact, pre2, mean2, rstd2, ctx_c, mask_i))
            if compact:
                h_next = ops.place_rows(h_next, rows_c.inv, M, ops.BF16_NAN_BITS)
            h = h_next

        ctx.model = model
        ctx.dims = (B, T, R, S, d, H, dh, nL)
        ctx.drop = (p_drop, p_attn, seed_step)
        ctx.u_holds_grad = nL > 0 and u_holds_grad
        ctx.rows_c = rows_c
        ctx.saved = (tok if text_embed is not None else x, totlen, rowmask, ximg16, loc, emb_saved, saved_layers)
        ctx.refine = (ref_saved, keylen_img, p_refine)
        ctx.input_grads = (R > 0 and x_img.requires_grad and track, text_embed is not None)
        ctx.langs = langs
        ctx.positions = positions
        ctx.h0_mode = None if h0 is None else h0.dtype
        hook = model.ddp_hook
        ctx.track = bool(track) and hook is not None
        ctx.tok_rows_max = hook.encoder_forward(0 if h0 is not None else T * B) if ctx.track else None
        ctx.set_materialize_grads(False)
        ctx.sink = GradSink()
        model._pending_sink = ctx.sink
        return h

    @staticmethod
    def backward(ctx, dout):
        model = ctx.model
        ar = model.arena()
        B, T, R, S, d, H, dh, nL = ctx.dims
        M = B * S
        p_drop, p_attn, seed_step = ctx.drop
        x, totlen, rowmask, ximg16, loc, emb_saved, saved_layers = ctx.saved
        ctx.saved = None
        rows_c = ctx.rows_c
        seed = lambda kind, i=0: rng.stream_seed(model.base_seed, seed_step, _site(kind, i))
        ref_saved, keylen_img, p_refine = ctx.refine
        ctx.refine = None
        hook = model.ddp_hook if ctx.track else None
        if model.ddp_hook is not None:
            model.ddp_hook.params_ready(None)
        sunk = ctx.sink.take()
        if dout is None and sunk is None:
            if hook is not None:
                hook.encoder_backward_end()
            return (None,) * N_ENC_ARGS
        if dout is None:
            dh_ = sunk
        else:
            dh_ = dout.contiguous()
            if dh_.dtype != BF16:
                dh_ = dh_.to(BF16)
            if sunk is not None:
                dh_ = dh_ + sunk.view_as(dh_)
        last = hook.encoder_backward_begin() if hook is not None else True
        st8 = model.fp8_state() if model.fp8 else None

        def dgrad(g, i, gsite, wsite, wt16, epi, pre8=None, **kw):
            if st8 is None or wsite not in fp8mod.BWD_SITES:
                return ops.gemm_nt(g, wt16, epi, **kw)
            g8, dgs = pre8 if pre8 is not None else st8.quant(g, i, gsite)
            _, wt8, dws = st8.weights[(i, wsite)]
            return ops.gemm_nt_fp8(g8, wt8, epi, a_is_bf8=True, descale_a=dgs, descale_b=dws, **kw)

        for i in reversed(range(nL)):
            a, f = 'attentions.%d.' % i, 'ffns.%d.' % i
            (h_in, qkv, ctxt, lse, pre1, mean1, rstd1, x1, u, hact, pre2, mean2, rstd2, ctx_c, mask_i) = saved_layers[i]
            saved_layers[i] = None
            compact = rows_c is not None and i == nL - 1
            rr = {}
            if compact:
                rr = dict(rng_rows=rows_c.idx)
                dh_ = ops.gather_rows(dh_.view(M, d), rows_c.idx, rows_c.n, d)
            dpre2, dY2 = ops.layernorm_bwd(dh_, None, pre2, ar.p('layer_norm2.%d.weight' % i), mean2, rstd2, mask_i,
                                           ar.g('layer_norm2.%d.weight' % i), ar.g('layer_norm2.%d.bias' % i),
                                           dbias_drop=ar.g(f + 'lin2.bias'), want_drop=p_drop > 0,
                                           seed=seed('ffn', i), p_drop=p_drop, **rr)
            if dY2 is None:
                dY2 = dpre2
            ops.gemm_wgrad(dY2, hact, ar.g(f + 'lin2.weight'))
            du8 = None
            if ctx.u_holds_grad == 'q':
                o8 = {}
                if st8 is not None and 'w1' in fp8mod.BWD_SITES:
                    kd = st8.index(i, 'du')
                    if st8.seen[kd]:
                        o8 = dict(out8=torch.empty((M, 4 * d), dtype=torch.uint8, device=dY2.device), scale8=st8.scale[kd:kd + 1],
                                  amax8=st8.amax[kd:kd + 1], out8_bf8=True)
                dU = ops.gemm_nt(dY2, ar.wt[('lin2', i)], L.EPI_MULQ, aux=u, colsum=ar.g(f + 'lin1.bias'), **o8)
                if o8:
                    du8 = (o8['out8'], st8.descale[kd:kd + 1])
                elif st8 is not None and 'w1' in fp8mod.BWD_SITES:
                    st8._first_use(dU, kd)
            else:
                dU = dgrad(dY2, i, 'dy2', 'w2', ar.wt[('lin2', i)], L.EPI_MUL if ctx.u_holds_grad else L.EPI_DGELU, aux=u,
                           colsum=ar.g(f + 'lin1.bias'))
            del hact, u, pre2
            ops.gemm_wgrad(dU, x1, ar.g(f + 'lin1.weight'))
            dx1 = dgrad(dU, i, 'du', 'w1', ar.wt[('lin1', i)], L.EPI_RES, aux=dpre2, pre8=du8)
            del dU, dpre2, dY2
            dpre1, dAO = ops.layernorm_bwd(dx1, None, pre1, ar.p('layer_norm1.%d.weight' % i), mean1, rstd1, None,
                                           ar.g('layer_norm1.%d.weight' % i), ar.g('layer_norm1.%d.bias' % i),
                                           dbias_drop=ar.g(a + 'out_lin.bias'), want_drop=p_drop > 0,
                                           seed=seed('attn_out', i), p_drop=p_drop, **rr)
            if dAO is None:
                dAO = dpre1
            dctx = dgrad(dAO, i, 'dao', 'wout', ar.wt[('out', i)], L.EPI_NONE)
            if compact:
                ops.gemm_wgrad(dAO, ctx_c, ar.g(a + 'out_lin.weight'))
                dctx = ops.place_rows(dctx, rows_c.inv, M, 0)
                dpre1 = ops.place_rows(dpre1, rows_c.inv, M, 0)
            dqkv = ops.attn_bwd(qkv, totlen, ctxt, dctx, lse[0], B, S, H, dh, dbias_qkv=ar.qkv_bias(i, grad=True),
                                seed=seed('attn_p', i), p_drop=p_attn, keepmask=lse[1])
            if compact:
                ops.gemm_wgrad(dqkv, h_in, ar.qkv_wgrad(i))
            else:
                ops.gemm_wgrad_pair(dqkv, h_in, ar.qkv_wgrad(i), dAO, ctxt, ar.g(a + 'out_lin.weight'))
            dh_ = dgrad(dqkv, i, 'dqkv', 'wqkv', ar.wt[('qkv', i)], L.EPI_RES, aux=dpre1)
            del dqkv, dctx, dAO, dpre1, dx1
            ar.touch_layer(i)
            if hook is not None:
                hook.layer_done(i, last)
        if ctx.h0_mode is not None:
            if hook is not None:
                hook.embed_done(last, ids=None, rows=None, n_max=ctx.tok_rows_max)
            return (None,) * 14 + (dh_.to(ctx.h0_mode), None, None)
        want_dximg, has_text_embed = ctx.input_grads
        langs, positions = ctx.langs, ctx.positions
        tok_rows = None
        if has_text_embed or langs is not None or positions is not None or (hook is not None and hook.active):
            tok_rows = torch.empty((T * B, d), dtype=BF16, device=dh_.device)
        grads = dict(
            d_g_emb=ar.g('layer_norm_emb.weight'), d_be_emb=ar.g('layer_norm_emb.bias'),
            d_pos=ar.g('position_embeddings.weight'), d_emb=ar.g('embeddings.weight'),
            d_g_img=ar.g('image_embeddings.LayerNorm.weight'), d_be_img=ar.g('image_embeddings.LayerNorm.bias'),
            d_b_img=ar.g('image_embeddings.image_embeddings.bias'),
            d_b_loc=ar.g('image_embeddings.image_location_embeddings.bias'),
            d_w_loc=ar.g('image_embeddings.image_location_embeddings.weight'))
        de = ops.embed_assemble_bwd(dh_, emb_saved, ar.p('layer_norm_emb.weight'),
                                    ar.p('image_embeddings.LayerNorm.weight'), x, totlen, loc, grads, B, T, R, d,
                                    -1 if has_text_embed else model.pad_index, seed_img=seed('img'), seed_emb=seed('emb'), p_drop=p_drop,
                                    img_rows_bwd=None if ref_saved is None else
                                    (lambda g: refiner_bwd(model, g, ref_saved, keylen_img, B, R, seed_step, p_refine)),
                                    tok_rows=tok_rows)
        ar.touch('layer_norm_emb.weight', 'layer_norm_emb.bias', 'position_embeddings.weight')
        if not has_text_embed:
            ar.touch('embeddings.weight')
        d_ximg = d_text = None
        if R > 0:
            ops.gemm_wgrad(de, ximg16, ar.g('image_embeddings.image_embeddings.weight'))
            ar.touch(*[n for n in ar.names if n.startswith('image_embeddings.')])
            if want_dximg:
                d_ximg = ops.gemm_nt(de, _transposed(ar.w('image_embeddings.image_embeddings.weight')), L.EPI_NONE)
                d_ximg = d_ximg.view(R, B, 2048).float()
        if has_text_embed:
            d_text = tok_rows.view(T, B, d).transpose(0, 1).float()
            tok_rows = None
        if langs is not None:
            npad = (model.n_langs + 7) // 8 * 8
            onehot = torch.zeros((T * B, npad), dtype=BF16, device=tok_rows.device)
            onehot.scatter_(1, langs.view(-1, 1), 1.0)
            dl = torch.zeros((npad, d), dtype=torch.float32, device=tok_rows.device)
            ops.gemm_wgrad(onehot, tok_rows, dl)
            ar.g('cross_lang_embeddings.weight').add_(dl[:model.n_langs])
            ar.touch('cross_lang_embeddings.weight')
        if positions is not None:
            gpos = ar.g('position_embeddings.weight')
            rows32 = tok_rows.float()
            gpos.index_add_(0, positions.reshape(-1), rows32)
            gpos[:T].sub_(rows32.view(T, B, d).sum(dim=1))
        if (langs is not None or positions is not None) and (hook is None or not hook.active):
            ops.scatter_add_token_rows(tok_rows, x.contiguous().view(-1), ar.g('embeddings.weight'), model.pad_index)
            tok_rows = None
        if hook is not None:
            hook.embed_done(last, ids=x if tok_rows is not None else None, rows=tok_rows, n_max=ctx.tok_rows_max)
        return (None, None, None, None, d_ximg, None, None, None, None, None, None, None, d_text, None, None, None, None)


class ImageStreamFn(torch.autograd.Function):

    @staticmethod
    def forward(ctx, anchor, model, x_img, lengths, image_loc, langs, p_drop, seed_step, p_refine=None, track=False):
        ar = model.arena()
        ar.refresh()
        dev = ar.device
        d = model.dim
        R, B = x_img.shape[0], x_img.shape[1]
        seed = lambda kind: rng.stream_seed(model.base_seed, seed_step, _site(kind))
        ximg16 = ops.cast_bf16(x_img.to(dev).contiguous().view(R * B, 2048))
        loc = image_loc.to(dev).contiguous().float()
        img_proj = ops.gemm_nt(ximg16, ar.w('image_embeddings.image_embeddings.weight'), L.EPI_BIAS,
                               bias=ar.p('image_embeddings.image_embeddings.bias'))
        rows, img_saved = ops.embed_image_rows_fwd(
            img_proj, loc, ar.p('image_embeddings.image_location_embeddings.weight'),
            ar.p('image_embeddings.image_location_embeddings.bias'), ar.p('image_embeddings.LayerNorm.weight'),
            ar.p('image_embeddings.LayerNorm.bias'), B, R, d, seed_img=seed('img'), p_drop=p_drop)
        if langs is not None:
            langs = langs.to(dev).contiguous()
            rows = (rows.float() + ar.p('cross_lang_embeddings.weight')[langs.t()].reshape(B * R, d)).to(BF16)
        totlen = lengths.to(device=dev, dtype=torch.int32).contiguous()
        mask = (torch.arange(R, device=dev, dtype=torch.int32)[None, :] < totlen[:, None]).reshape(B * R, 1)
        h0 = ops.dropout_rows(rows, p_drop, seed('emb')) * mask.to(BF16)
        ref_saved = None
        if p_refine is not None:
            h0, ref_saved = refiner_fwd(model, h0.contiguous(), totlen, B, R, seed_step, p_refine)
        ctx.model = model
        ctx.saved = (ximg16, loc, img_saved, totlen, mask, langs, ref_saved)
        ctx.meta = (B, R, d, p_drop, seed_step, p_refine)
        ctx.x_img_meta = (x_img.dtype, x_img.device) if x_img.requires_grad else None
        ctx.hook = model.ddp_hook if track else None
        if ctx.hook is not None:
            ctx.hook.stream_forward()
        return h0

    @staticmethod
    def backward(ctx, dh0):
        model = ctx.model
        ar = model.arena()
        ximg16, loc, img_saved, totlen, mask, langs, ref_saved = ctx.saved
        ctx.saved = None
        B, R, d, p_drop, seed_step, p_refine = ctx.meta
        seed = lambda kind: rng.stream_seed(model.base_seed, seed_step, _site(kind))
        if ref_saved is not None:
            dh0 = refiner_bwd(model, dh0.to(BF16).contiguous(), ref_saved, totlen, B, R, seed_step, p_refine)
            ar.touch(*[n for n in ar.names if n.startswith('refine_embeddings.')])
        g = (dh0.to(BF16) * mask.to(BF16)).contiguous()
        d_rows = ops.dropout_rows(g, p_drop, seed('emb'))
        if langs is not None:
            npad = (model.n_langs + 7) // 8 * 8
            onehot = torch.zeros((B * R, npad), dtype=BF16, device=g.device)
            onehot.scatter_(1, langs.t().reshape(-1, 1), 1.0)
            dl = torch.zeros((npad, d), dtype=torch.float32, device=g.device)
            ops.gemm_wgrad(onehot, d_rows, dl)
            ar.g('cross_lang_embeddings.weight').add_(dl[:model.n_langs])
            ar.touch('cross_lang_embeddings.weight')
        grads = dict(d_g_img=ar.g('image_embeddings.LayerNorm.weight'), d_be_img=ar.g('image_embeddings.LayerNorm.bias'),
                     d_b_img=ar.g('image_embeddings.image_embeddings.bias'),
                     d_b_loc=ar.g('image_embeddings.image_location_embeddings.bias'),
                     d_w_loc=ar.g('image_embeddings.image_location_embeddings.weight'))
        de = ops.embed_image_rows_bwd(d_rows, img_saved, ar.p('image_embeddings.LayerNorm.weight'), loc, totlen, grads, B, R, d,
                                      seed_img=seed('img'), p_drop=p_drop)
        ops.gemm_wgrad(de, ximg16, ar.g('image_embeddings.image_embeddings.weight'))
        ar.touch(*[n for n in ar.names if n.startswith('image_embeddings.')])
        d_ximg = None
        if ctx.x_img_meta is not None:
            d_rows = ops.gemm_nt(de, _transposed(ar.w('image_embeddings.image_embeddings.weight')), L.EPI_NONE)
            d_ximg = d_rows.view(R, B, 2048).to(device=ctx.x_img_meta[1], dtype=ctx.x_img_meta[0])
        if ctx.hook is not None:
            ctx.hook.stream_backward_end()
        return (None, None, d_ximg) + (None,) * 7


N_DEC_ARGS = 12

CAUSAL_TILED_MIN_T = 32

CROSS_TILED_MIN_TQ = 8
CROSS_TILED_MIN_S = 36


# ... 610 lines not shown
```

### m3p_amd/lib.py

```python
import ctypes as C
import os

import torch

_HERE = os.path.dirname(os.path.abspath(__file__))
LIB_PATH = os.environ.get('M3P_HIP_LIB') or os.path.join(_HERE, 'libm3p_hip.so')

EPI_NONE, EPI_BIAS, EPI_BIAS_GELU, EPI_BIAS_DROP_RES, EPI_RES, EPI_DGELU, EPI_MUL, EPI_MULQ, EPI_BIAS_GELUQ, EPI_BIAS_LSE = range(10)
KERN_NT_SKINNY, KERN_NT_W8, KERN_NT_W8_QUEUE, KERN_NT_W4, KERN_NT_RING, KERN_NT_128 = range(1, 7)
KERN_WGRAD_W4_CHUNKS, KERN_WGRAD_W4_TILES, KERN_WGRAD_RING, KERN_WGRAD_128 = range(10, 14)


class M3PError(RuntimeError):
    pass


class Epilogue(C.Structure):
    _fields_ = [
        ('bias', C.c_void_p), ('aux', C.c_void_p), ('out2', C.c_void_p), ('colsum', C.c_void_p),
        ('ld_aux', C.c_int32), ('ld_out2', C.c_int32), ('scale_cols', C.c_int32), ('scale', C.c_float),
        ('alpha', C.c_float), ('seed', C.c_uint32), ('thresh24', C.c_uint32), ('inv_keep', C.c_float),
        ('descale_a', C.c_void_p), ('descale_b', C.c_void_p),
        ('out8', C.c_void_p), ('scale8', C.c_void_p), ('amax8', C.c_void_p), ('ld_out8', C.c_int32), ('out8_bf8', C.c_int32),
        ('rng_rows', C.c_void_p),
        ('row_ref', C.c_void_p),
    ]


_p, _i, _f, _u32 = C.c_void_p, C.c_int, C.c_float, C.c_uint32

SIGNATURES = {
    'm3p_version': (C.c_char_p, []),
    'm3p_gemm_nt_bf16': (_i, [_p, _i, _p, _i, _p, _i, _i, _i, _i, _i, C.POINTER(Epilogue), _p]),
    'm3p_gemm_nt_fp8': (_i, [_p, _i, _i, _p, _i, _p, _i, _i, _i, _i, _i, C.POINTER(Epilogue), _p]),
    'm3p_quant_fp8': (_i, [_p, _i, _p, _i, _i, _i, _p, _p, _i, _p]),
    'm3p_quant_fp8_batch': (_i, [_p, _i, _i, _p]),
    'm3p_gemm_nt_streamk_f32': (_i, [_p, _i, _p, _i, _p, _i, _i, _i, _i, _f, _p]),
    'm3p_gemm_nn_streamk_f32': (_i, [_p, _i, _p, _i, _i, _p, _i, _i, _i, _i, _f, _p]),
    'm3p_gemm_nn_w4_f32': (_i, [_p, _i, _p, _i, _p, _i, _i, _i, _i, _f, _p, C.c_size_t, _p]),
    'm3p_gemm_wgrad_workspace_bytes': (C.c_size_t, []),
    'm3p_gemm_wgrad_bf16': (_i, [_p, _i, _p, _i, _p, _i, _i, _i, _i, _f, _p, C.c_size_t, _p]),
    'm3p_gemm_wgrad_store_bf16': (_i, [_p, _i, _p, _i, _p, _i, _i, _i, _i, _f, _p, C.c_size_t, _p]),
    'm3p_gemm_wgrad_pair_bf16': (_i, [_p, _i, _p, _i, _p, _i, _i, _i, _p, _i, _p, _i, _p, _i, _i, _i, _i, _f, _p, C.c_size_t, _p]),
    'm3p_layernorm_fwd': (_i, [_p, _p, _p, _p, _p, _p, _p, _i, _i, _f, _p]),
    'm3p_layernorm_bwd': (_i, [_p, _p, _p, _p, _p, _p, _p, _p, _p, _p, _p, _p, _i, _i, _u32, _u32, _f, _p]),
    'm3p_layernorm_bwd_rows': (_i, [_p, _p, _p, _p, _p, _p, _p, _p, _p, _p, _p, _p, _i, _i, _u32, _u32, _f, _p, _p]),
    'm3p_attn_fwd': (_i, [_p, _p, _p, _p, _p, _i, _i, _i, _i, _u32, _u32, _f, _p]),
    'm3p_attn_bwd': (_i, [_p, _p, _p, _p, _p, _p, _p, _p, _i, _i, _i, _i, _f, _u32, _u32, _f, _p]),
    'm3p_attn_query_fwd': (_i, [_p, _i, _p, C.c_longlong, _i, _p, _p, _i, _i, _i, _i, _i, _i, _i, _p]),
    'm3p_attn_query_owner_fwd': (_i, [_p, _i, _p, C.c_longlong, _i, _p, _p, _i, _i, _i, _i, _i, _i, _i, _p, _i, _i, _p]),
    'm3p_vocab_select_max_k': (_i, []),
    'm3p_vocab_select_plan': (_i, [_i, _i, _i, _i, _i]),
    'm3p_vocab_select_workspace_bytes': (C.c_size_t, [_i, _i, _i]),
    'm3p_vocab_select': (_i, [_p, _i, _i, _i, _p, _i, _i, _p, C.c_size_t, _p, _p, _p, _p]),
    'm3p_vocab_sample_plan': (_i, [_i, _i, _i, _i]),
    'm3p_vocab_sample_workspace_bytes': (C.c_size_t, [_i, _i, _i]),
    'm3p_vocab_sample': (_i, [_p, _i, _i, _i, _f, _i, _u32, _p, C.c_size_t, _p, _p, _p, _p]),
    'm3p_attn_rows_fwd': (_i, [_p, _i, _p, C.c_longlong, _i, _p, _p, _p, _i, _i, _i, _i, _i, _i, _i, _u32, _u32, _f, _p]),
    'm3p_attn_rows_bwd': (_i, [_p, _i, _p, C.c_longlong, _i, _p, _p, _p, _p, _i, _p, _i, _i, _i, _i, _i, _i, _i, _f, _u32, _u32, _f, _p]),
    'm3p_attn_causal_fwd': (_i, [_p, _i, _p, _p, _i, _i, _i, _i, _u32, _u32, _f, _p]),
    'm3p_attn_causal_bwd': (_i, [_p, _i, _p, _p, _p, _i, _i, _i, _i, _i, _f, _u32, _u32, _f, _p]),
    'm3p_attn_cross_fwd': (_i, [_p, _i, _p, C.c_longlong, _i, _p, _p, _p, _i, _i, _i, _i, _i, _u32, _u32, _f, _p]),
    'm3p_attn_cross_bwd': (_i, [_p, _i, _p, C.c_longlong, _i, _p, _p, _p, _p, _i, _p, _i, _i, _i, _i, _i, _i, _f, _u32, _u32, _f, _p]),
    'm3p_cast_f32_bf16': (_i, [_p, _p, C.c_longlong, _p]),
    'm3p_embed_assemble_fwd': (_i, [_p] * 19 + [_i, _i, _i, _i, _u32, _u32, _u32, _f, _p, _p]),
    'm3p_embed_image_rows_fwd': (_i, [_p] * 10 + [_i, _i, _i, _u32, _u32, _f, _p]),
    'm3p_embed_assemble_bwd': (_i, [_p] * 24 + [_i, _i, _i, _i, _i, _u32, _u32, _u32, _f, _i, _p]),
    'm3p_dropout_rows': (_i, [_p, _i, _p, _i, _p, _i, _i, _i, _u32, _u32, _u32, _u32, _f, _p]),
    'm3p_glu_fwd': (_i, [_p, _i, _p, _i, _i, _p]),
    'm3p_glu_bwd': (_i, [_p, _i, _p, _p, _i, _i, _p]),
    'm3p_gather_rows': (_i, [_p, _p, _p, _i, _i, _p]),
    'm3p_place_rows': (_i, [_p, _p, _p, _i, _i, _i, _u32, _p]),
    'm3p_scatter_add_rows': (_i, [_p, _p, _p, _i, _i, _p]),
    'm3p_scatter_add_token_rows': (_i, [_p, _i, _p, _p, _i, _i, _i, _p]),
    'm3p_ce_fwd_bwd': (_i, [_p, _i, _i, _i, _p, _p, _p, _f, _f, _p]),
    'm3p_ce_colsum_workspace_bytes': (C.c_size_t, [_i, _i]),
    'm3p_ce_fwd_bwd_colsum': (_i, [_p, _i, _i, _i, _p, _p, _p, _f, _p, _p, C.c_size_t, _p]),
    'm3p_ce_lse_from_blocks': (_i, [_p, _i, _i, _p, _i, _p, _p, _p, _p, _p]),
    'm3p_ce_bwd_colsum': (_i, [_p, _i, _i, _i, _p, _p, _f, _p, _p, C.c_size_t, _p]),
    'm3p_ce_shift_target': (_i, [_p, _p, _p, _p, _p, _p, _i, _i, _p]),
    'm3p_ce_shift_rows': (_i, [_p, _i, _i, _f, _p, _p, _p, _p, _p]),
    'm3p_ce_shift_colsum': (_i, [_p, _i, _i, _p, _p, _p, C.c_size_t, _p]),
    'm3p_ce_shift_scale_rows': (_i, [_p, _p, _p, _p, _i, _i, _p]),
    'm3p_ce_shift_target_rows': (_i, [_p, _p, _p, _p, _p, _p, _i, _i, _p]),
    'm3p_ce_shift_dh': (_i, [_p, _p, _p, _p, _p, _p, _p, _i, _i, _p]),
    'm3p_ce_eval': (_i, [_p, _i, _i, _i, _p, _p, _p, _p]),
    'm3p_colsum_bf16': (_i, [_p, _i, _i, _i, _p, _p, _p]),
    'm3p_sumsq_f32': (_i, [_p, C.c_longlong, _p, _p]),
    'm3p_sumsq_ranges_f32': (_i, [_p, _p, _p, _i, _p, _p]),
    'm3p_adam_step': (_i, [_p, _p, _p, _p, _p, C.c_longlong, _f, _f, _f, _f, _f, _f, _p, _f, _f, _i, _p]),
    'm3p_adam_step_ranges': (_i, [_p, _p, _p, _p, _p, _p, _p, _p, _p, _i, _f, _f, _f, _f, _f, _p, _f, _f, _p]),
    'm3p_itm_score_fwd': (_i, [_p, _p, _p, _p, _p, _i, _i, _p]),
    'm3p_itm_score_bwd': (_i, [_p, _p, _p, _p, _p, _i, _p, _p, _p, _i, _i, _p]),
    'm3p_gelu_bwd': (_i, [_p, _p, _p, C.c_longlong, _p]),
    'm3p_mse_fwd_bwd': (_i, [_p, _i, _p, _i, _p, _p, _i, _i, _f, _p]),
    'm3p_gelu_fwd': (_i, [_p, _p, _p, C.c_longlong, _p]),
    'm3p_gelu_fwd_gq': (_i, [_p, _p, _p, _i, _i, _p]),
    'm3p_gelu_fwd_q8': (_i, [_p, _p, _p, C.c_longlong, _p, _p, _p]),
    'm3p_transpose_batch_bf16': (_i, [_p, _i, _i, _p]),
    'm3p_transpose_bf16': (_i, [_p, _p, _i, _i, _i, _i, _p]),
    'm3p_set_persistent_grid': (_i, [_i]),
    'm3p_set_tile_queue': (_i, [_p, _i]),
    'm3p_gemm_nt_plan': (_i, [_i, _i, _i, _i]),
    'm3p_gemm_wgrad_plan': (_i, [_i, _i, _i]),
    'm3p_debug_set_variant': (None, [_i]),
    'm3p_debug_attn_variant': (None, [_i]),
    'm3p_seq_masks': (_i, [_p, _p, _i, _i, _p, _p, _p]),
    'm3p_mask_to_rows': (_i, [_p, _i, _i, C.c_longlong, C.c_longlong, C.c_longlong, _i, _p, _i, _p]),
    'm3p_cast_rows_f32_bf16': (_i, [_p, C.c_longlong, C.c_longlong, _i, _i, _i, _p, _p]),
    'm3p_scale_bf16_dev': (_i, [_p, _i, _p, _p, C.c_longlong, _p]),
    'm3p_axpy_dev_f32': (_i, [_p, _p, _p, C.c_longlong, _p]),
    'm3p_itm_loss_fwd_bwd': (_i, [_p, _p, _i, _i, _f, _f, _p, _p, _p]),
    'm3p_probe_mfma_16x16x32': (_i, [_p, _p, _p, _p, _p]),
    'm3p_probe_mfma_fp8_16x16x128': (_i, [_p, _p, _p, _i, _p]),
    'm3p_probe_tr16': (_i, [_p, _p, _p]),
    'm3p_probe_permlane16_swap': (_i, [_p, _p]),
}

_lib = None


def load():
    global _lib
    if _lib is not None:
        return _lib
    if not os.path.exists(LIB_PATH):
        raise M3PError('libm3p_hip.so not found at %s — build it first (make -C m3p_amd/csrc); '
                       'there is no fallback path' % LIB_PATH)
    lib = C.CDLL(LIB_PATH)
    for name, (res, args) in SIGNATURES.items():
        fn = getattr(lib, name)
        fn.restype = res
        fn.argtypes = args
    _lib_tq = os.environ.get('M3P_TILE_QUEUE', '0') != '0'
    _lib = lib
    if _lib_tq and torch.cuda.is_available():
        from . import ops
        ops.set_tile_queue(True)
    return lib


def check(code, what):
    if code != 0:
        kind = {-1: 'M3P_EINVAL (bad shape/alignment)', -2: 'M3P_ENOTIMPL', -3: 'M3P_ENOMEM'}.get(code, 'hipError_t %d' % code)
        raise M3PError('%s failed: %s' % (what, kind))


def ptr(t):
    return None if t is None else t.data_ptr()


def stream():
    return torch.cuda.current_stream().cuda_stream


def num_cus():
    n = torch.cuda.get_device_properties(torch.cuda.current_device()).multi_processor_count
    return max(n - n % 8, 8)


def thresh24(p):
    return int(round(float(p) * (1 << 24)))
```

### m3p_amd/ops.py

```python
import ctypes as C
import os

import torch

from . import lib as L
from . import rng

BF16 = torch.bfloat16
_DEBUG_CHECKS = os.environ.get('M3P_DEBUG_CHECKS') == '1'

PROFILE = None
_EPI_NAMES = ['gemm_nt/none', 'gemm_nt/bias', 'gemm_nt/bias_gelu', 'gemm_nt/bias_drop_res', 'gemm_nt/res',
              'gemm_nt/dgelu', 'gemm_nt/mul', 'gemm_nt/mulq', 'gemm_nt/bias_geluq', 'gemm_nt/bias_lse']


PROFILE_ONLY = None


def _prof_begin(key=None):
    if PROFILE is None or (PROFILE_ONLY is not None and key != PROFILE_ONLY):
        return None
    e = torch.cuda.Event(enable_timing=True)
    e.record()
    return e
# ... 120 lines not shown
    _chk_bf16(a, w)
    M, K = a.shape
    N = w.shape[0]
    assert w.shape[1] == K and out_f32.dtype == torch.float32 and out_f32.shape == (M, N)
    e0 = _prof_begin(('gemm_nt/streamk', M, N, K))
    rc = L.load().m3p_gemm_nt_streamk_f32(a.data_ptr(), a.stride(0), w.data_ptr(), w.stride(0), out_f32.data_ptr(),
                                          out_f32.stride(0), M, N, K, alpha, L.stream())
    L.check(rc, 'm3p_gemm_nt_streamk_f32')
    _prof_end(e0, ('gemm_nt/streamk', M, N, K))
    return out_f32


def gemm_nn_streamk(a, w_kn, out_f32, alpha=1.0):
    _chk_bf16(a, w_kn)
    M, K = a.shape
    k_valid, N = w_kn.shape
    assert k_valid <= K and out_f32.dtype == torch.float32 and out_f32.shape == (M, N) and w_kn.stride(1) == 1
    e0 = _prof_begin(('gemm_nt/streamk', M, N, K))
    rc = L.load().m3p_gemm_nn_streamk_f32(a.data_ptr(), a.stride(0), w_kn.data_ptr(), w_kn.stride(0), k_valid,
                                          out_f32.data_ptr(), out_f32.stride(0), M, N, K, alpha, L.stream())
    L.check(rc, 'm3p_gemm_nn_streamk_f32')
    _prof_end(e0, ('gemm_nt/streamk', M, N, K))
    return out_f32


def gemm_nn(a, w_kn, out_f32, alpha=1.0, k_rows_readable=None):
    _chk_bf16(a, w_kn)
    M, K = a.shape
    k_valid, N = w_kn.shape
    if (k_rows_readable or k_valid) >= K and M % 256 == 0 and N % 256 == 0 and K % 64 == 0 and K >= 4096:
        assert out_f32.dtype == torch.float32 and out_f32.shape == (M, N) and w_kn.stride(1) == 1
        e0 = _prof_begin(('gemm_nn/w4', M, N, K))
        ws = _wgrad_workspace(a.device)
        rc = L.load().m3p_gemm_nn_w4_f32(a.data_ptr(), a.stride(0), w_kn.data_ptr(), w_kn.stride(0), out_f32.data_ptr(),
                                         out_f32.stride(0), M, N, K, alpha, ws.data_ptr(), ws.numel(), L.stream())
        if rc == 0:
            _prof_end(e0, ('gemm_nn/w4', M, N, K))
            return out_f32
        if rc != -2:
            L.check(rc, 'm3p_gemm_nn_w4_f32')
    return gemm_nn_streamk(a, w_kn, out_f32, alpha)


_WGRAD_WS = {}


def _wgrad_workspace(device):
    key = (device.index, torch.cuda.current_stream(device).cuda_stream)
    ws = _WGRAD_WS.get(key)
    if ws is None:
        ws = _WGRAD_WS[key] = torch.empty(int(L.load().m3p_gemm_wgrad_workspace_bytes()), dtype=torch.uint8, device=device)
    return ws


def gemm_wgrad(dy, x, dw, alpha=1.0, n=None, k=None, dw_is_zero=False, report_store=False, must_store=False):
    _chk_bf16(dy, x)
    assert dw.dtype == torch.float32 and dw.stride(-1) == 1
    M = dy.shape[0]
    N = dy.shape[1] if n is None else n
    K = x.shape[1] if k is None else k
    assert x.shape[0] == M and dw.shape[0] >= N and dw.shape[1] >= K
    e0 = _prof_begin(('gemm_wgrad', M, N, K))
    ws = _wgrad_workspace(dy.device)
    if dw_is_zero:
        rc = L.load().m3p_gemm_wgrad_store_bf16(dy.data_ptr(), dy.stride(0), x.data_ptr(), x.stride(0), dw.data_ptr(),
                                                dw.stride(0), M, N, K, alpha, ws.data_ptr(), ws.numel(), L.stream())
        if rc == 0:
            _prof_end(e0, ('gemm_wgrad', M, N, K))
            return True if report_store else dw
        if rc != -2:
            L.check(rc, 'm3p_gemm_wgrad_store_bf16')
        if must_store:
            raise L.M3PError('m3p_gemm_wgrad_store_bf16 declined (M3P_ENOTIMPL) a store the caller depends on: dw is not physically zero')
    rc = L.load().m3p_gemm_wgrad_bf16(dy.data_ptr(), dy.stride(0), x.data_ptr(), x.stride(0), dw.data_ptr(),
                                      dw.stride(0), M, N, K, alpha, ws.data_ptr(), ws.numel(), L.stream())
    L.check(rc, 'm3p_gemm_wgrad_bf16')
    _prof_end(e0, ('gemm_wgrad', M, N, K))
    return False if report_store else dw


def gemm_wgrad_pair(dy_a, x_a, dw_a, dy_b, x_b, dw_b, alpha=1.0):
    _chk_bf16(dy_a, x_a, dy_b, x_b)
    assert dw_a.dtype == torch.float32 and dw_b.dtype == torch.float32 and dw_a.stride(-1) == 1 and dw_b.stride(-1) == 1
    M = dy_a.shape[0]
    assert x_a.shape[0] == M and dy_b.shape[0] == M and x_b.shape[0] == M
    Na, Ka, Nb, Kb = dy_a.shape[1], x_a.shape[1], dy_b.shape[1], x_b.shape[1]
    assert dw_a.shape[0] >= Na and dw_a.shape[1] >= Ka and dw_b.shape[0] >= Nb and dw_b.shape[1] >= Kb
    e0 = _prof_begin(('gemm_wgrad_pair', M, Na + Nb, Ka))
    ws = _wgrad_workspace(dy_a.device)
    rc = L.load().m3p_gemm_wgrad_pair_bf16(dy_a.data_ptr(), dy_a.stride(0), x_a.data_ptr(), x_a.stride(0), dw_a.data_ptr(), dw_a.stride(0),
                                           Na, Ka, dy_b.data_ptr(), dy_b.stride(0), x_b.data_ptr(), x_b.stride(0), dw_b.data_ptr(),
                                           dw_b.stride(0), Nb, Kb, M, alpha, ws.data_ptr(), ws.numel(), L.stream())
    L.check(rc, 'm3p_gemm_wgrad_pair_bf16')
    _prof_end(e0, ('gemm_wgrad_pair', M, Na + Nb, Ka))


def layernorm_fwd(x, gamma, beta, rowmask=None, eps=1e-12):
    _chk_bf16(x)
    rows, d = x.shape
    assert x.is_contiguous()
    y = torch.empty_like(x)
    mean = torch.empty(rows, dtype=torch.float32, device=x.device)
    rstd = torch.empty(rows, dtype=torch.float32, device=x.device)
    rc = L.load().m3p_layernorm_fwd(x.data_ptr(), gamma.data_ptr(), beta.data_ptr(), L.ptr(rowmask), y.data_ptr(),
                                    mean.data_ptr(), rstd.data_ptr(), rows, d, eps, L.stream())
    L.check(rc, 'm3p_layernorm_fwd')
    return y, mean, rstd


def layernorm_bwd(dy_a, dy_b, x, gamma, mean, rstd, rowmask, dgamma, dbeta, dbias_drop=None,
                  want_drop=False, seed=0, p_drop=0.0, rng_rows=None):
    _chk_bf16(dy_a, dy_b, x)
    rows, d = x.shape
    if rng_rows is not None:
        assert rng_rows.dtype == torch.int32 and rng_rows.is_cuda and rng_rows.is_contiguous() and rng_rows.numel() == rows
    dx = torch.empty_like(x)
    dx_drop = torch.empty_like(x) if want_drop else None
    rc = L.load().m3p_layernorm_bwd_rows(dy_a.data_ptr(), L.ptr(dy_b), x.data_ptr(), gamma.data_ptr(), mean.data_ptr(),
                                         rstd.data_ptr(), L.ptr(rowmask), dx.data_ptr(), L.ptr(dx_drop),
                                         dgamma.data_ptr(), dbeta.data_ptr(), L.ptr(dbias_drop), rows, d, seed,
                                         L.thresh24(p_drop), 1.0 / (1.0 - p_drop) if p_drop > 0 else 1.0,
                                         L.ptr(rng_rows), L.stream())
    L.check(rc, 'm3p_layernorm_bwd_rows')
    return dx, dx_drop


def attn_fwd(qkv, keylen, B, S, H, dh, seed=0, p_drop=0.0, want_mask=False):
    _chk_bf16(qkv)
    assert qkv.is_contiguous() and qkv.shape == (B * S, 3 * H * dh) and keylen.dtype == torch.int32
    ctx = torch.empty((B * S, H * dh), dtype=BF16, device=qkv.device)
    lse = torch.empty((B, H, S), dtype=torch.float32, device=qkv.device)
    mask = None
    if want_mask and p_drop > 0:
        nt = (S + 15) // 16
        mask = torch.empty((B * H, nt, nt, 4), dtype=torch.int64, device=qkv.device)
    rc = L.load().m3p_attn_fwd(qkv.data_ptr(), keylen.data_ptr(), ctx.data_ptr(), lse.data_ptr(), L.ptr(mask), B, S, H, dh,
                               seed, L.thresh24(p_drop), 1.0 / (1.0 - p_drop) if p_drop > 0 else 1.0, L.stream())
    L.check(rc, 'm3p_attn_fwd')
    return (ctx, lse, mask) if want_mask else (ctx, lse)


def attn_bwd(qkv, keylen, ctx, dctx, lse, B, S, H, dh, dbias_qkv=None, seed=0, p_drop=0.0, keepmask=None):
    _chk_bf16(qkv, ctx, dctx)
    assert dctx.is_contiguous() and ctx.is_contiguous()
    assert p_drop == 0 or keepmask is not None, 'attention backward with dropout needs the keep words of the forward pass'
    dqkv = torch.empty_like(qkv)
    rc = L.load().m3p_attn_bwd(qkv.data_ptr(), keylen.data_ptr(), ctx.data_ptr(), dctx.data_ptr(), lse.data_ptr(),
                               L.ptr(keepmask), dqkv.data_ptr(), L.ptr(dbias_qkv), B, S, H, dh, 1.0 / (dh ** 0.5), seed,
                               L.thresh24(p_drop), 1.0 / (1.0 - p_drop) if p_drop > 0 else 1.0, L.stream())
    L.check(rc, 'm3p_attn_bwd')
    return dqkv


def attn_query_fwd(q, kv, klen, B, Tq, H, dh, Lk, causal=False, pos0=0, owner=None):
    _chk_bf16(q, kv)
    assert q.stride(1) == 1 and kv.dim() == 3 and kv.stride(2) == 1 and kv.shape[1] >= Lk
    ctx = torch.empty((B * Tq, H * dh), dtype=BF16, device=q.device)
    if owner is None:
        assert kv.shape[0] == B
        rc = L.load().m3p_attn_query_fwd(q.data_ptr(), q.stride(0), kv.data_ptr(), kv.stride(0), kv.stride(1), L.ptr(klen),
                                         ctx.data_ptr(), B, Tq, H, dh, Lk, 1 if causal else 0, pos0, L.stream())
        L.check(rc, 'm3p_attn_query_fwd')
        return ctx
    assert owner.dtype == torch.int32 and owner.is_cuda and owner.shape[0] == B and owner.dim() in (1, 2)
    assert owner.dim() == 1 or (owner.shape[1] >= Lk and owner.stride(1) == 1)
    if _DEBUG_CHECKS:
        used = owner if owner.dim() == 1 else owner[:, :Lk]
        assert int(used.min()) >= 0 and int(used.max()) < kv.shape[0], 'owner names a row outside the key / value tensor'
    rc = L.load().m3p_attn_query_owner_fwd(q.data_ptr(), q.stride(0), kv.data_ptr(), kv.stride(0), kv.stride(1), L.ptr(klen),
                                           ctx.data_ptr(), B, Tq, H, dh, Lk, 1 if causal else 0, pos0, owner.data_ptr(),
                                           owner.stride(0), 1 if owner.dim() == 2 else 0, L.stream())
    L.check(rc, 'm3p_attn_query_owner_fwd')
    return ctx


_ENOTIMPL = -2


def vocab_select_max_k():
    return int(L.load().m3p_vocab_select_max_k())


def vocab_select_takes(n, V, ld, beam, k):
    rc = L.load().m3p_vocab_select_plan(n, V, ld, beam, k)
    if rc == _ENOTIMPL:
        return False
    L.check(rc, 'm3p_vocab_select_plan')
    return True


def vocab_select(logits, V, beam_scores, beam, k):
    _chk_bf16(logits)
    assert logits.dim() == 2 and logits.stride(1) == 1
    n = logits.shape[0]
    assert n % beam == 0 and logits.shape[1] >= V
    if beam_scores is not None:
        assert beam_scores.dtype == torch.float32 and beam_scores.is_cuda and beam_scores.is_contiguous() and beam_scores.numel() == n
    lib = L.load()
    rc = lib.m3p_vocab_select_plan(n, V, logits.stride(0), beam, k)
    if rc == _ENOTIMPL:
        return None
    L.check(rc, 'm3p_vocab_select_plan')
    bs = n // beam
    dev = logits.device
    ws_bytes = lib.m3p_vocab_select_workspace_bytes(n, V, k)
    ws = torch.empty((ws_bytes,), dtype=torch.uint8, device=dev)
    scores = torch.empty((bs, k), dtype=torch.float32, device=dev)
    flat_idx = torch.empty((bs, k), dtype=torch.int64, device=dev)
    lse = torch.empty((n,), dtype=torch.float32, device=dev)
    rc = lib.m3p_vocab_select(logits.data_ptr(), logits.stride(0), n, V, L.ptr(beam_scores), beam, k, ws.data_ptr(), ws_bytes,
                              scores.data_ptr(), flat_idx.data_ptr(), lse.data_ptr(), L.stream())
    L.check(rc, 'm3p_vocab_select')
    return scores, flat_idx, lse


def vocab_sample_takes(n, V, ld, top_k):
    rc = L.load().m3p_vocab_sample_plan(n, V, ld, top_k)
    if rc == _ENOTIMPL:
        return False
    L.check(rc, 'm3p_vocab_sample_plan')
    return True


def vocab_sample(logits, V, temperature, seed, top_k=0):
    _chk_bf16(logits)
    assert logits.dim() == 2 and logits.stride(1) == 1 and logits.shape[1] >= V
    n = logits.shape[0]
    lib = L.load()
    rc = lib.m3p_vocab_sample_plan(n, V, logits.stride(0), top_k)
    if rc == _ENOTIMPL:
        return None
    L.check(rc, 'm3p_vocab_sample_plan')
    dev = logits.device
    ws_bytes = lib.m3p_vocab_sample_workspace_bytes(n, V, top_k)
    ws = torch.empty((ws_bytes,), dtype=torch.uint8, device=dev)
    words = torch.empty((n,), dtype=torch.int64, device=dev)
    logprob = torch.empty((n,), dtype=torch.float32, device=dev)
    key = torch.empty((n,), dtype=torch.float32, device=dev)
    rc = lib.m3p_vocab_sample(logits.data_ptr(), logits.stride(0), n, V, rng.inv_temperature(temperature), top_k,
                              int(seed) & 0xFFFFFFFF, ws.data_ptr(), ws_bytes, words.data_ptr(), logprob.data_ptr(), key.data_ptr(),
                              L.stream())
    L.check(rc, 'm3p_vocab_sample')
    return words, logprob, key


def attn_rows_fwd(q, kv, klen, B, Tq, H, dh, Lk, causal=False, seed=0, p_drop=0.0):
    _chk_bf16(q, kv)
    assert q.stride(1) == 1 and kv.dim() == 3 and kv.stride(2) == 1 and kv.shape[0] == B and kv.shape[1] >= Lk
    ctx = torch.empty((B * Tq, H * dh), dtype=BF16, device=q.device)
    lse = torch.empty((B, H, Tq), dtype=torch.float32, device=q.device)
    rc = L.load().m3p_attn_rows_fwd(q.data_ptr(), q.stride(0), kv.data_ptr(), kv.stride(0), kv.stride(1), L.ptr(klen),
                                    ctx.data_ptr(), lse.data_ptr(), B, Tq, H, dh, Lk, 1 if causal else 0, 0, seed,
                                    L.thresh24(p_drop), 1.0 / (1.0 - p_drop) if p_drop > 0 else 1.0, L.stream())
    L.check(rc, 'm3p_attn_rows_fwd')
    return ctx, lse


def attn_rows_bwd(q, kv, klen, dctx, lse, B, Tq, H, dh, Lk, qscale, causal=False, seed=0, p_drop=0.0, dq_out=None):
    _chk_bf16(q, kv, dctx)
    assert dctx.is_contiguous()
    d = H * dh
    dq = dq_out if dq_out is not None else torch.empty((B * Tq, d), dtype=BF16, device=q.device)
    dkv = torch.zeros((B, Lk, 2 * d), dtype=torch.float32, device=q.device)
    rc = L.load().m3p_attn_rows_bwd(q.data_ptr(), q.stride(0), kv.data_ptr(), kv.stride(0), kv.stride(1), L.ptr(klen),
                                    dctx.data_ptr(), lse.data_ptr(), dq.data_ptr(), dq.stride(0), dkv.data_ptr(), B, Tq, H, dh, Lk,
                                    1 if causal else 0, 0, qscale, seed, L.thresh24(p_drop),
                                    1.0 / (1.0 - p_drop) if p_drop > 0 else 1.0, L.stream())
    L.check(rc, 'm3p_attn_rows_bwd')
    return dq, dkv


def _attn_tiled_fwd_out(out, B, T, H, dh, device):
    if out is None:
        return (torch.empty((B * T, H * dh), dtype=BF16, device=device), torch.empty((B, H, T), dtype=torch.float32, device=device))
    ctx, lse = out
    assert ctx.dtype == BF16 and ctx.is_contiguous() and ctx.shape == (B * T, H * dh)
    assert lse.dtype == torch.float32 and lse.is_contiguous() and lse.shape == (B, H, T)
    return ctx, lse


def attn_causal_fwd(qkv, B, T, H, dh, seed=0, p_drop=0.0, out=None):
    _chk_bf16(qkv)
    assert qkv.dim() == 2 and qkv.stride(1) == 1 and qkv.shape[0] == B * T and qkv.shape[1] >= 3 * H * dh
    ctx, lse = _attn_tiled_fwd_out(out, B, T, H, dh, qkv.device)
    th, ik = _drop_args(p_drop)
    rc = L.load().m3p_attn_causal_fwd(qkv.data_ptr(), qkv.stride(0), ctx.data_ptr(), lse.data_ptr(), B, T, H, dh, seed, th, ik,
                                      L.stream())
    if rc == -2:
        return None
    L.check(rc, 'm3p_attn_causal_fwd')
    return ctx, lse


def attn_causal_bwd(qkv, dctx, lse, B, T, H, dh, qscale, seed=0, p_drop=0.0, out=None):
    _chk_bf16(qkv, dctx)
    assert qkv.dim() == 2 and qkv.stride(1) == 1 and qkv.shape[0] == B * T and dctx.is_contiguous()
    assert dctx.shape == (B * T, H * dh) and lse.dtype == torch.float32 and lse.is_contiguous() and lse.shape == (B, H, T)
    if out is not None:
        dqkv = out
        assert dqkv.dtype == BF16 and dqkv.stride(1) == 1 and dqkv.shape == (B * T, 3 * H * dh)
    else:
        dqkv = torch.empty((B * T, 3 * H * dh), dtype=BF16, device=qkv.device)
    th, ik = _drop_args(p_drop)
    rc = L.load().m3p_attn_causal_bwd(qkv.data_ptr(), qkv.stride(0), dctx.data_ptr(), lse.data_ptr(), dqkv.data_ptr(),
                                      dqkv.stride(0), B, T, H, dh, qscale, seed, th, ik, L.stream())
    if rc == -2:
# ... 545 lines not shown
```

Baseline: 8072 sequences/s.

## Compute last-layer attention only for compacted query rows via listed kernels

In the last layer, where only the masked/target rows are needed, queries are projected and attended only for a compact list of rows, while K/V are still computed for all positions. This uses new listed forward and backward attention kernels that index queries through per-batch offset and entry lists. The aim is to cut Q-projection, attention and gather work down to the needed rows. It adds separate split Q and KV GEMMs and a scatter-add in the backward pass, and is limited to the shape with dh=64 and S of 161 to 176.

```diff
diff --git a/include/m3p_hip.h b/include/m3p_hip.h
--- a/include/m3p_hip.h
+++ b/include/m3p_hip.h
@@ -107,6 +107,14 @@
                          int H, int dh, float qscale, uint32_t seed, uint32_t thresh24, float inv_keep,
                          void* stream);
 
+M3P_API int m3p_attn_fwd_listed(const void* q, const void* kv, int ld_kv, const int32_t* keylen, const int32_t* q_off,
+                                const int32_t* q_ent, int n, void* ctx, float* lse, uint64_t* keepmask, int B, int S, int H,
+                                int dh, uint32_t seed, uint32_t thresh24, float inv_keep, void* stream);
+M3P_API int m3p_attn_bwd_listed(const void* q, const void* kv, int ld_kv, const int32_t* keylen, const int32_t* q_off,
+                                const int32_t* q_ent, int n, const void* ctx, const void* dctx, const float* lse,
+                                const uint64_t* keepmask, void* dq, void* dkv, int ld_dkv, float* dbias_qkv, int B, int S, int H,
+                                int dh, float qscale, uint32_t thresh24, float inv_keep, void* stream);
+
 M3P_API int m3p_attn_query_fwd(const void* q, int ld_q, const void* kv, long long kv_bstride, int ld_kv,
                                const int32_t* klen, void* ctx, int B, int Tq, int H, int dh, int Lk, int causal,
                                int pos0, void* stream);
diff --git a/m3p_amd/csrc/attention.hip b/m3p_amd/csrc/attention.hip
--- a/m3p_amd/csrc/attention.hip
+++ b/m3p_amd/csrc/attention.hip
@@ -99,11 +99,21 @@
   }
 }
 
-template <int DH, int KT, bool DROP, int NTC, int NW = 4, bool EVENS = false>
+struct QueryList {
+  const bf16* q;
+  const int* q_off;
+  const int* q_ent;
+  int n, ld_kv;
+};
+__device__ __forceinline__ int list_entry(const QueryList& ql, int q0, int nq, int j) {
+  return ql.q_ent[min(q0 + max(min(j, nq - 1), 0), ql.n - 1)];
+}
+
+template <int DH, int KT, bool DROP, int NTC, int NW = 4, bool EVENS = false, bool LIST = false>
 __global__ __launch_bounds__(NW * 64, NW == 8 ? 2 : 3)
 void attn_fwd_kernel(const bf16* __restrict__ qkv, const int* __restrict__ keylen, bf16* __restrict__ ctx,
                      float* __restrict__ lse, unsigned long long* __restrict__ keepmask, int S, int H, int dmodel,
-                     uint32_t seed, uint32_t thresh24, float inv_keep) {
+                     uint32_t seed, uint32_t thresh24, float inv_keep, QueryList ql) {
   using Cf = AttnCfg<DH>;
   extern __shared__ __attribute__((aligned(16))) char smem[];
   const int tid = threadIdx.x, lane = tid & 63;
@@ -111,10 +121,17 @@
   const int b = blockIdx.x / H, h = blockIdx.x - b * H;
   const int nt = NTC ? NTC : (S + 15) >> 4;
   const int nk = (nt + 1) >> 1;
-  const size_t ld = 3 * (size_t)dmodel;
-  const bf16* Qg = qkv + (size_t)b * S * ld + h * DH;
-  const bf16* Kg = Qg + dmodel;
-  const bf16* Vg = Qg + 2 * dmodel;
+  const size_t ld = LIST ? (size_t)ql.ld_kv : 3 * (size_t)dmodel;
+  const size_t ldq = LIST ? (size_t)dmodel : ld;
+  const bf16* Qg = LIST ? ql.q + h * DH : qkv + (size_t)b * S * ld + h * DH;
+  const bf16* Kg = LIST ? qkv + (size_t)b * S * ld + h * DH : Qg + dmodel;
+  const bf16* Vg = Kg + dmodel;
+  int q0 = 0, nq = S;
+  if (LIST) {
+    q0 = ql.q_off[b];
+    nq = min(ql.q_off[b + 1] - q0, S);
+  }
+  const int nqt = LIST ? (nq + 15) >> 4 : nt;
   char* sK = smem;
   char* sV = smem + nt * 16 * Cf::ROWB;
   stage_rows<DH>(Kg, ld, S, nt * 16, sK, wid, lane, NW);
@@ -122,11 +139,16 @@
   const int fq = lane & 15, fg = lane >> 4;
   const int wrot = (wid + (blockIdx.x >> 3)) & (NW - 1);
   bf16x8 qnext[Cf::KK];
+  int entn = 0;
   {
-    const int qc0 = min(wrot * 16 + fq, S - 1);
+    int qc0 = min(wrot * 16 + fq, S - 1);
+    if (LIST) {
+      entn = list_entry(ql, q0, nq, wrot * 16 + fq);
+      qc0 = entn >> 9;
+    }
 #pragma unroll
     for (int kk = 0; kk < Cf::KK; ++kk)
-      qnext[kk] = *reinterpret_cast<const bf16x8*>(Qg + (size_t)qc0 * ld + 32 * kk + 8 * fg);
+      qnext[kk] = *reinterpret_cast<const bf16x8*>(Qg + (size_t)qc0 * ldq + 32 * kk + 8 * fg);
   }
   const int klen = keylen[b];
   __syncthreads();
@@ -140,17 +162,22 @@
   for (int n = 0; n < Cf::NT; ++n)
     v_off[n] = vrow * Cf::ROWB + Cf::swz(2 * n + ((fq & 3) >> 1), vrow) * 16 + 8 * (fq & 1);
 
-  for (int qb = wrot; qb < nt; qb += NW) {
+  for (int qb = wrot; qb < nqt; qb += NW) {
     const int q = qb * 16 + fq;
-    const int qc = min(q, S - 1);
+    const int ent = entn;
+    const int qc = LIST ? (ent & 511) : min(q, S - 1);
     bf16x8 qf[Cf::KK];
 #pragma unroll
     for (int kk = 0; kk < Cf::KK; ++kk) qf[kk] = qnext[kk];
     {
-      const int qcn = min(q + 16 * NW, S - 1);
+      int qcn = min(q + 16 * NW, S - 1);
+      if (LIST) {
+        entn = list_entry(ql, q0, nq, q + 16 * NW);
+        qcn = entn >> 9;
+      }
 #pragma unroll
       for (int kk = 0; kk < Cf::KK; ++kk)
-        qnext[kk] = *reinterpret_cast<const bf16x8*>(Qg + (size_t)qcn * ld + 32 * kk + 8 * fg);
+        qnext[kk] = *reinterpret_cast<const bf16x8*>(Qg + (size_t)qcn * ldq + 32 * kk + 8 * fg);
     }
 
     f32x4 s[2 * KT];
@@ -283,8 +310,13 @@
       bf16x4 ob[Cf::NT];
 #pragma unroll
       for (int n = 0; n < Cf::NT; ++n) ob[n] = bf16x4{(bf16)o[n][0], (bf16)o[n][1], (bf16)o[n][2], (bf16)o[n][3]};
+      if (LIST) {
+        store_row_widened<Cf::NT>(ctx + (size_t)(ent >> 9) * dmodel + h * DH, fg, q < nq, ob);
+        if (q < nq && fg == 0) lse[(size_t)h * ql.n + (ent >> 9)] = mx + __logf(sum);
+      } else {
       store_row_widened<Cf::NT>(ctx + (size_t)(b * S + min(q, S - 1)) * dmodel + h * DH, fg, q < S, ob);
       if (q < S && fg == 0) lse[(size_t)(b * H + h) * S + q] = mx + __logf(sum);
+      }
     }
   }
 }
@@ -800,12 +832,13 @@
 
 #undef PAD_TILE
 
-template <bool DROP, bool MASK>
-__global__ __launch_bounds__(768, 3)
-void attn_bwd_p_kernel(const bf16* __restrict__ qkv, const int* __restrict__ keylen, const bf16* __restrict__ ctx,
-                       const bf16* __restrict__ dctx, const float* __restrict__ lse,
-                       const unsigned long long* __restrict__ keepmask, bf16* __restrict__ dqkv,
-                       float* __restrict__ dbias_qkv, int S, int H, int dmodel, int nheads, float qscale, float inv_keep) {
+template <bool DROP, bool MASK, bool LIST>
+__device__ __forceinline__
+void attn_bwd_p_body(const bf16* __restrict__ qkv, const int* __restrict__ keylen, const bf16* __restrict__ ctx,
+                     const bf16* __restrict__ dctx, const float* __restrict__ lse,
+                     const unsigned long long* __restrict__ keepmask, bf16* __restrict__ dqkv,
+                     float* __restrict__ dbias_qkv, int S, int H, int dmodel, int nheads, float qscale, float inv_keep,
+                     const QueryList& ql, bf16* __restrict__ dq_list, int ld_dkv) {
   constexpr int DH = 64, NW = 12, NKC = 6, NTC = 11, NR = NKC * 32;
   using Cf = AttnCfg<DH>;
   constexpr int DSP = NTC * 32;
@@ -821,7 +854,7 @@
   float* sD = sL + NR;
   float* sB = sD + NR;
   unsigned long long* sMW = reinterpret_cast<unsigned long long*>(sB + 2 * NW * 3 * DH) + wid * 48;
-  const size_t ld = 3 * (size_t)dmodel;
+  const size_t ld = LIST ? (size_t)ql.ld_kv : 3 * (size_t)dmodel;
   const int fq = lane & 15, fg = lane >> 4;
   const int rin = lane / Cf::CH, c8 = lane % Cf::CH;
   int r_off[Cf::KK];
@@ -845,6 +878,41 @@
   unsigned long long mw_req = 0;
   auto request_head = [&](int hd) {
     const int b = hd / H, h = hd - b * H;
+    if constexpr (LIST) {
+      const int q0 = ql.q_off[b];
+      const int nq = min(ql.q_off[b + 1] - q0, NTC * 16);
+      const int nrows = ((nq + 31) >> 5) * 32;
+      int ent_st[kNIW];
+#pragma unroll
+      for (int j = 0; j < kNIW; ++j) ent_st[j] = list_entry(ql, q0, nq, (wid + j * NW) * Cf::RPI + rin);
+      const int ent_l = list_entry(ql, q0, nq, tid);
+      const bf16* Kh = qkv + (size_t)b * S * ld + h * DH;
+      const int keyc = min(min(wid, NTC - 1) * 16 + fq, S - 1);
+#pragma unroll
+      for (int kk = 0; kk < Cf::KK; ++kk) {
+        kf[kk] = *reinterpret_cast<const bf16x8*>(Kh + (size_t)keyc * ld + 32 * kk + 8 * fg);
+        vf[kk] = *reinterpret_cast<const bf16x8*>(Kh + dmodel + (size_t)keyc * ld + 32 * kk + 8 * fg);
+      }
+      const uint32_t lds_q = (uint32_t)(uintptr_t)(__attribute__((address_space(3))) char*)s0;
+      const uint32_t lds_d = (uint32_t)(uintptr_t)(__attribute__((address_space(3))) char*)s1;
+#pragma unroll
+      for (int j = 0; j < kNIW; ++j) {
+        const int i = wid + j * NW;
+        orow[j] = bf16x8{0, 0, 0, 0, 0, 0, 0, 0};
+        if (i * Cf::RPI < nrows) {
+          const int row = i * Cf::RPI + rin;
+          const size_t at = (size_t)(ent_st[j] >> 9) * dmodel + h * DH + Cf::swz(c8, row) * 8;
+          orow[j] = *reinterpret_cast<const bf16x8*>(ctx + at);
+          const bf16* src_q = ql.q + at;
+          const bf16* src_d = dctx + at;
+          const uint32_t dst_q = __builtin_amdgcn_readfirstlane(lds_q + (uint32_t)i * 1024u);
+          const uint32_t dst_d = __builtin_amdgcn_readfirstlane(lds_d + (uint32_t)i * 1024u);
+          asm volatile("s_mov_b32 m0, %1\n\ts_nop 0\n\tglobal_load_lds_dwordx4 %0, off" :: "v"(src_q), "s"(dst_q) : "memory", "m0");
+          asm volatile("s_mov_b32 m0, %1\n\ts_nop 0\n\tglobal_load_lds_dwordx4 %0, off" :: "v"(src_d), "s"(dst_d) : "memory", "m0");
+        }
+      }
+      if (tid < nq) lse_r = lse[(size_t)h * ql.n + (ent_l >> 9)];
+    } else {
     const bf16* Qg = qkv + (size_t)b * S * ld + h * DH;
     const bf16* Og = ctx + (size_t)b * S * dmodel + h * DH;
     const bf16* dOg = dctx + (size_t)b * S * dmodel + h * DH;
@@ -862,6 +930,7 @@
       vf[kk] = *reinterpret_cast<const bf16x8*>(Qg + 2 * dmodel + (size_t)keyc * ld + 32 * kk + 8 * fg);
     }
     if (tid < NR && tid < S) lse_r = lse[(size_t)hd * S + tid];
+    }
     if (MASK && lane < 4 * NTC)
       mw_req = keepmask[(size_t)hd * NTC * NTC * 4 + ((size_t)(lane >> 2) * NTC + min(wid, NTC - 1)) * 4 + (lane & 3)];
   };
@@ -913,12 +982,21 @@
   bf16x4 kb4[Cf::NT], vb4[Cf::NT], qb4[Cf::NT];
   const int key = wid * 16 + fq;
   bf16* dQg_prev = nullptr;
+  int par = 0, prev_h = -1;
+  int ent_prev = 0, nq_prev = 0;
   auto store_head = [&](bf16* dQh) {
     if (wid < NTC) {
+      if constexpr (LIST) {
+        bf16* row = dQh + (size_t)min(key, S - 1) * ld_dkv;
+        store_row_widened<Cf::NT>(dq_list + (size_t)(ent_prev >> 9) * dmodel + prev_h * DH, fg, key < nq_prev, qb4);
+        store_row_widened<Cf::NT>(row, fg, key < S, kb4);
+        store_row_widened<Cf::NT>(row + dmodel, fg, key < S, vb4);
+      } else {
       bf16* row = dQh + (size_t)min(key, S - 1) * ld;
       store_row_widened<Cf::NT>(row, fg, key < S, qb4);
       store_row_widened<Cf::NT>(row + dmodel, fg, key < S, kb4);
       store_row_widened<Cf::NT>(row + 2 * dmodel, fg, key < S, vb4);
+      }
     }
   };
   int hd = blockIdx.x;
@@ -926,12 +1004,17 @@
   constexpr int kStagger = 2;
   for (int i = 0; i < (int)((blockIdx.x >> 3) & 3) * kStagger; ++i) __builtin_amdgcn_s_sleep(16);
   request_head(hd);
-  int par = 0, prev_h = -1;
   for (;;) {
     const int b = hd / H, h = hd - b * H;
-    bf16* dQg = dqkv + (size_t)b * S * ld + h * DH;
-    const bf16* Kg = qkv + (size_t)b * S * ld + h * DH + dmodel;
+    bf16* dQg = LIST ? dqkv + (size_t)b * S * ld_dkv + h * DH : dqkv + (size_t)b * S * ld + h * DH;
+    const bf16* Kg = qkv + (size_t)b * S * ld + h * DH + (LIST ? 0 : dmodel);
     const int klen = keylen[b];
+    int q0 = 0, nq = S;
+    if (LIST) {
+      q0 = ql.q_off[b];
+      nq = min(ql.q_off[b + 1] - q0, NTC * 16);
+    }
+    const int nkq = LIST ? (nq + 31) >> 5 : NKC, nqt = LIST ? (nq + 15) >> 4 : NTC;
     float* sBh = sB + par * (NW * 3 * DH);
     __builtin_amdgcn_s_waitcnt(0x0F70);
     asm volatile("s_waitcnt vmcnt(0)" ::: "memory");
@@ -945,10 +1028,10 @@
         for (int e = 0; e < 8; ++e) part += (float)orow[j][e] * (float)dvv[e];
         part = chunks_sum<Cf::CH>(part);
         const int row = i * Cf::RPI + rin;
-        if (c8 == 0) sD[row] = row < S ? part * keep_prob : 0.f;
-      }
-    }
-    if (tid < NR) sL[tid] = tid < S ? lse_r * kLog2e - log2_inv_keep : INFINITY;
+        if (c8 == 0) sD[row] = row < nq ? part * keep_prob : 0.f;
+      }
+    }
+    if (tid < NR) sL[tid] = tid < nq ? lse_r * kLog2e - log2_inv_keep : INFINITY;
     if (MASK && lane < 4 * NTC) sMW[lane] = mw_req;
     asm volatile("s_waitcnt lgkmcnt(0)" ::: "memory");
     __builtin_amdgcn_s_barrier();
@@ -956,6 +1039,10 @@
     if (prev_h >= 0 && dbias_qkv) bias_reduce(sB + (par ^ 1) * (NW * 3 * DH), prev_h);
     if (prev_h >= 0) store_head(dQg_prev);
     dQg_prev = dQg;
+    if (LIST) {
+      ent_prev = list_entry(ql, q0, nq, key);
+      nq_prev = nq;
+    }
     stage_rows_hidden<DH>(Kg, ld, S, NR, sK, wid, lane, NW);
     if (wid < NTC) {
       const float kbias = (key < klen) ? 0.f : kMasked;
@@ -964,6 +1051,7 @@
       for (int n = 0; n < Cf::NT; ++n) dv[n] = dk[n] = f32x4{0.f, 0.f, 0.f, 0.f};
 #pragma unroll
       for (int kq = 0; kq < NKC; ++kq) {
+        if (LIST && kq >= nkq) break;
         f32x4 scA[2], dpA[2], dnegA[2];
 #pragma unroll
         for (int hf = 0; hf < 2; ++hf) {
@@ -1043,7 +1131,7 @@
     asm volatile("" ::: "memory");
     const int next = hd + gridDim.x;
     if (next < nheads) request_head(next);
-    if (wid < NTC) {
+    if (wid < nqt) {
       f32x4 dq[Cf::NT];
 #pragma unroll
       for (int n = 0; n < Cf::NT; ++n) dq[n] = f32x4{0.f, 0.f, 0.f, 0.f};
@@ -1063,7 +1151,7 @@
 #pragma unroll
       for (int n = 0; n < Cf::NT; ++n) {
         qb4[n] = bf16x4{(bf16)(dq[n][0] * qscale), (bf16)(dq[n][1] * qscale), (bf16)(dq[n][2] * qscale), (bf16)(dq[n][3] * qscale)};
-        if (dbias_qkv) bias_acc(n, key < S ? qb4[n] : bf16x4{0, 0, 0, 0});
+        if (dbias_qkv) bias_acc(n, key < nq ? qb4[n] : bf16x4{0, 0, 0, 0});
       }
     }
     if (dbias_qkv) bias_flush(sBh + wid * 3 * DH, 0);
@@ -1078,6 +1166,27 @@
     bias_reduce(sB + (par ^ 1) * (NW * 3 * DH), prev_h);
   }
 #undef PAD_TILE
+}
+
+template <bool DROP, bool MASK>
+__global__ __launch_bounds__(768, 3)
+void attn_bwd_p_kernel(const bf16* __restrict__ qkv, const int* __restrict__ keylen, const bf16* __restrict__ ctx,
+                       const bf16* __restrict__ dctx, const float* __restrict__ lse,
+                       const unsigned long long* __restrict__ keepmask, bf16* __restrict__ dqkv,
+                       float* __restrict__ dbias_qkv, int S, int H, int dmodel, int nheads, float qscale, float inv_keep) {
+  attn_bwd_p_body<DROP, MASK, false>(qkv, keylen, ctx, dctx, lse, keepmask, dqkv, dbias_qkv, S, H, dmodel, nheads, qscale, inv_keep,
+                                     QueryList{}, nullptr, 0);
+}
+
+template <bool DROP, bool MASK>
+__global__ __launch_bounds__(768, 3)
+void attn_bwd_pl_kernel(const bf16* __restrict__ kv, const int* __restrict__ keylen, const bf16* __restrict__ ctx,
+                        const bf16* __restrict__ dctx, const float* __restrict__ lse,
+                        const unsigned long long* __restrict__ keepmask, bf16* __restrict__ dkv,
+                        float* __restrict__ dbias_qkv, int S, int H, int dmodel, int nheads, float qscale, float inv_keep,
+                        QueryList ql, bf16* __restrict__ dq_list, int ld_dkv) {
+  attn_bwd_p_body<DROP, MASK, true>(kv, keylen, ctx, dctx, lse, keepmask, dkv, dbias_qkv, S, H, dmodel, nheads, qscale, inv_keep, ql,
+                                    dq_list, ld_dkv);
 }
 
 template <int DH>
@@ -1096,13 +1205,27 @@
     hipError_t e = hipFuncSetAttribute((const void*)kern, hipFuncAttributeMaxDynamicSharedMemorySize, (int)lds); \
     if (e != hipSuccess) return (int)e;                                                                         \
     hipLaunchKernelGGL(kern, dim3(B* H), dim3((wide || NW0 == 8) ? 512 : 256), lds, st, qkv, keylen, ctx, lse, keepmask, S, H, dmodel, seed, \
-                       thresh24, inv_keep);                                                                     \
+                       thresh24, inv_keep, QueryList{});                                                        \
   } while (0)
   if (nk <= 6) M3P_ATTN_FWD(6);
   else if (nk <= 12) M3P_ATTN_FWD(12);
   else if (nk <= 16) M3P_ATTN_FWD(16);
   else return M3P_EINVAL;
 #undef M3P_ATTN_FWD
+  M3P_CHECK_LAUNCH();
+  return M3P_OK;
+}
+
+int launch_fwd_listed(const bf16* kv, const int* keylen, bf16* ctx, float* lse, unsigned long long* keepmask, int B, int S, int H,
+                      int dmodel, uint32_t seed, uint32_t thresh24, float inv_keep, const QueryList& ql, hipStream_t st) {
+  constexpr int DH = 64;
+  const int nt = (S + 15) / 16, nk = (S + 31) / 32;
+  if (nt != 11 || nk != 6 || (S & 1)) return M3P_ENOTIMPL;
+  const size_t lds = (size_t)(nt * 16 + nk * 32) * DH * 2;
+  auto kern = thresh24 ? attn_fwd_kernel<DH, 6, true, 11, 4, true, true> : attn_fwd_kernel<DH, 6, false, 11, 4, false, true>;
+  hipError_t e = hipFuncSetAttribute((const void*)kern, hipFuncAttributeMaxDynamicSharedMemorySize, (int)lds);
+  if (e != hipSuccess) return (int)e;
+  hipLaunchKernelGGL(kern, dim3(B * H), dim3(256), lds, st, kv, keylen, ctx, lse, keepmask, S, H, dmodel, seed, thresh24, inv_keep, ql);
   M3P_CHECK_LAUNCH();
   return M3P_OK;
 }
@@ -1155,6 +1278,24 @@
   return M3P_OK;
 }
 
+int launch_bwd_listed(const bf16* kv, const int* keylen, const bf16* ctx, const bf16* dctx, const float* lse,
+                      const unsigned long long* keepmask, bf16* dq, bf16* dkv, int ld_dkv, float* dbias, int B, int S, int H,
+                      int dmodel, float qscale, uint32_t thresh24, float inv_keep, const QueryList& ql, hipStream_t st) {
+  if ((S + 15) / 16 != 11 || (S + 31) / 32 != 6) return M3P_ENOTIMPL;
+  int dev = 0, n_cu = 0;
+  if (hipGetDevice(&dev) != hipSuccess || hipDeviceGetAttribute(&n_cu, hipDeviceAttributeMultiprocessorCount, dev) != hipSuccess || n_cu <= 0)
+    n_cu = 256;
+  const size_t ldsp = (size_t)3 * 192 * 128 + (size_t)11 * 16 * 11 * 32 + 2 * 192 * sizeof(float) + 2 * 12 * 3 * 64 * sizeof(float) + 12 * 48 * 8;
+  auto kp = thresh24 ? attn_bwd_pl_kernel<true, true> : attn_bwd_pl_kernel<false, false>;
+  hipError_t e = hipFuncSetAttribute((const void*)kp, hipFuncAttributeMaxDynamicSharedMemorySize, (int)ldsp);
+  if (e != hipSuccess) return (int)e;
+  const int nheads = B * H;
+  hipLaunchKernelGGL(kp, dim3(nheads < n_cu ? nheads : n_cu), dim3(768), ldsp, st, kv, keylen, ctx, dctx, lse, keepmask, dkv, dbias,
+                     S, H, dmodel, nheads, qscale, inv_keep, ql, dq, ld_dkv);
+  M3P_CHECK_LAUNCH();
+  return M3P_OK;
+}
+
 }
 
 extern "C" {
@@ -1189,4 +1330,35 @@
   return M3P_EINVAL;
 }
 
-}
+int m3p_attn_fwd_listed(const void* q, const void* kv, int ld_kv, const int32_t* keylen, const int32_t* q_off, const int32_t* q_ent,
+                        int n, void* ctx, float* lse, uint64_t* keepmask, int B, int S, int H, int dh, uint32_t seed,
+                        uint32_t thresh24, float inv_keep, void* stream) {
+  if (B <= 0 || S <= 0 || H <= 0 || n <= 0 || !q || !kv || !q_off || !q_ent || !ctx || !lse || !keylen) return M3P_EINVAL;
+  if (dh != 64) return M3P_ENOTIMPL;
+  const int dmodel = H * dh;
+  if (ld_kv < 2 * dmodel || (ld_kv % 8) != 0 || ((uintptr_t)q & 15) || ((uintptr_t)kv & 15) || ((uintptr_t)ctx & 15)) return M3P_EINVAL;
+  const QueryList ql{(const bf16*)q, q_off, q_ent, n, ld_kv};
+  return launch_fwd_listed((const bf16*)kv, keylen, (bf16*)ctx, lse, (unsigned long long*)keepmask, B, S, H, dmodel, seed, thresh24,
+                           inv_keep, ql, (hipStream_t)stream);
+}
+
+int m3p_attn_bwd_listed(const void* q, const void* kv, int ld_kv, const int32_t* keylen, const int32_t* q_off, const int32_t* q_ent,
+                        int n, const void* ctx, const void* dctx, const float* lse, const uint64_t* keepmask, void* dq, void* dkv,
+                        int ld_dkv, float* dbias_qkv, int B, int S, int H, int dh, float qscale, uint32_t thresh24, float inv_keep,
+                        void* stream) {
+  if (B <= 0 || S <= 0 || H <= 0 || n <= 0 || !q || !kv || !q_off || !q_ent || !ctx || !dctx || !lse || !dq || !dkv || !keylen)
+    return M3P_EINVAL;
+  if (thresh24 && !keepmask) return M3P_EINVAL;
+  if (dh != 64) return M3P_ENOTIMPL;
+  const int dmodel = H * dh;
+  if (ld_kv < 2 * dmodel || (ld_kv % 8) != 0 || ld_dkv < 2 * dmodel || (ld_dkv % 8) != 0) return M3P_EINVAL;
+  if (((uintptr_t)q & 15) || ((uintptr_t)kv & 15) || ((uintptr_t)ctx & 15) || ((uintptr_t)dctx & 15) || ((uintptr_t)dq & 15) ||
+      ((uintptr_t)dkv & 15))
+    return M3P_EINVAL;
+  const QueryList ql{(const bf16*)q, q_off, q_ent, n, ld_kv};
+  return launch_bwd_listed((const bf16*)kv, keylen, (const bf16*)ctx, (const bf16*)dctx, lse, (const unsigned long long*)keepmask,
+                           (bf16*)dq, (bf16*)dkv, ld_dkv, dbias_qkv, B, S, H, dmodel, qscale, thresh24, inv_keep, ql,
+                           (hipStream_t)stream);
+}
+
+}
diff --git a/m3p_amd/functional.py b/m3p_amd/functional.py
--- a/m3p_amd/functional.py
+++ b/m3p_amd/functional.py
@@ -433,6 +433,16 @@
     return n if (n >= COMPACT_MIN_ROWS and 2 * n <= M) else 0
 
 
+def query_lists(rows, S, B):
+    rows = torch.as_tensor(rows).long().cpu()
+    assert S <= 512 and rows.numel() < (1 << 22) and (rows.numel() == 0 or (int(rows.min()) >= 0 and int(rows.max()) < B * S))
+    seq, pos = rows // S, rows % S
+    order = torch.sort(seq, stable=True).indices
+    q_off = torch.zeros(B + 1, dtype=torch.int64)
+    q_off[1:] = torch.cumsum(torch.bincount(seq, minlength=B), 0)
+    return q_off.to(torch.int32), ((order << 9) | pos[order]).to(torch.int32)
+
+
 class OutputRows:
 
     def __init__(self, flags):
@@ -462,6 +472,17 @@
         if region_labels is not None and R > 0:
             flags[:, :R] |= torch.as_tensor(region_labels).cpu().reshape(B, R) != -1
         return cls(flags)
+
+    def query_list(self, S, device):
+        if not self.n or S > 512 or self.M % S or self.n >= (1 << 22):
+            return None
+        cache = self.__dict__.setdefault('_qlists', {})
+        key = (S, torch.device(device))
+        if key not in cache:
+            from .utils import to_cuda
+            with torch.cuda.device(device):
+                cache[key] = tuple(to_cuda(*query_lists(self._host[0], S, self.M // S)))
+        return cache[key]
 
     def to(self, device):
         if self.n and self.idx is None:
@@ -575,21 +596,32 @@
                 and ops.gq_eligible(M, 4 * d) == ops.gq_eligible(out_rows.n, 4 * d):
             assert out_rows.M == M, 'out_rows was built for %d rows, this pass has %d' % (out_rows.M, M)
             rows_c = out_rows.to(dev)
+        qlist = rows_c.query_list(S, dev) if rows_c is not None and ops.attn_listed_eligible(S, dh) else None
 
         for i in range(nL):
             a, f = 'attentions.%d.' % i, 'ffns.%d.' % i
             ready(('layer', i))
-            qkv = lin(h, i, 'x', 'wqkv', ar.qkv_w16(i), L.EPI_BIAS, bias=ar.qkv_bias(i), scale_cols=d, scale=qscale)
-            ctxt, lse, kmask = ops.attn_fwd(qkv, totlen, B, S, H, dh, seed=seed('attn_p', i), p_drop=p_attn,
-                                            want_mask=True)
-            lse = (lse, kmask)
             compact = rows_c is not None and i == nL - 1
-            Mi, ctx_in, res_in, mask_i, rr, ctx_c = M, ctxt, h, rowmask, {}, None
+            Mi, res_in, mask_i, rr, ctx_c = M, h, rowmask, {}, None
             if compact:
                 Mi, rr = rows_c.n, dict(rng_rows=rows_c.idx)
-                ctx_in = ctx_c = ops.gather_rows(ctxt, rows_c.idx, Mi, d)
                 res_in = ops.gather_rows(h, rows_c.idx, Mi, d)
                 mask_i = rowmask[rows_c.idx64]
+            if compact and qlist is not None:
+                w_qkv, b_qkv = ar.qkv_w16(i), ar.qkv_bias(i)
+                kv = ops.gemm_nt(h, w_qkv[d:], L.EPI_BIAS, bias=b_qkv[d:])
+                q_c = ops.gemm_nt(res_in, w_qkv[:d], L.EPI_BIAS, bias=b_qkv[:d], scale_cols=d, scale=qscale)
+                ctx_c, lse, kmask = ops.attn_fwd_listed(q_c, kv, totlen, qlist[0], qlist[1], B, S, H, dh,
+                                                        seed=seed('attn_p', i), p_drop=p_attn)
+                qkv, ctxt, ctx_in, ctx_c = (q_c, kv), None, ctx_c, (ctx_c, res_in)
+            else:
+                qkv = lin(h, i, 'x', 'wqkv', ar.qkv_w16(i), L.EPI_BIAS, bias=ar.qkv_bias(i), scale_cols=d, scale=qscale)
+                ctxt, lse, kmask = ops.attn_fwd(qkv, totlen, B, S, H, dh, seed=seed('attn_p', i), p_drop=p_attn,
+                                                want_mask=True)
+                ctx_in = ctxt
+                if compact:
+                    ctx_in = ctx_c = ops.gather_rows(ctxt, rows_c.idx, Mi, d)
+            lse = (lse, kmask)
             pre1 = lin(ctx_in, i, 'ctx', 'wout', ar.w(a + 'out_lin.weight'), L.EPI_BIAS_DROP_RES, bias=ar.p(a + 'out_lin.bias'),
                        aux=res_in, seed=seed('attn_out', i), p_drop=p_drop, **rr)
             x1, mean1, rstd1 = ops.layernorm_fwd(pre1, ar.p('layer_norm1.%d.weight' % i), ar.p('layer_norm1.%d.bias' % i))
@@ -638,6 +670,7 @@
         ctx.drop = (p_drop, p_attn, seed_step)
         ctx.u_holds_grad = nL > 0 and u_holds_grad
         ctx.rows_c = rows_c
+        ctx.qlist = qlist
         ctx.saved = (tok if text_embed is not None else x, totlen, rowmask, ximg16, loc, emb_saved, saved_layers)
         ctx.refine = (ref_saved, keylen_img, p_refine)
         ctx.input_grads = (R > 0 and x_img.requires_grad and track, text_embed is not None)
@@ -661,7 +694,7 @@
         p_drop, p_attn, seed_step = ctx.drop
         x, totlen, rowmask, ximg16, loc, emb_saved, saved_layers = ctx.saved
         ctx.saved = None
-        rows_c = ctx.rows_c
+        rows_c, qlist = ctx.rows_c, ctx.qlist
         seed = lambda kind, i=0: rng.stream_seed(model.base_seed, seed_step, _site(kind, i))
         ref_saved, keylen_img, p_refine = ctx.refine
         ctx.refine = None
@@ -734,6 +767,22 @@
             if dAO is None:
                 dAO = dpre1
             dctx = dgrad(dAO, i, 'dao', 'wout', ar.wt[('out', i)], L.EPI_NONE)
+            if compact and qlist is not None:
+                ctx_c, h_c = ctx_c
+                q_c, kv = qkv
+                dq_c, dkv = ops.attn_bwd_listed(q_c, kv, totlen, qlist[0], qlist[1], ctx_c, dctx, lse[0], B, S, H, dh,
+                                                dbias_qkv=ar.qkv_bias(i, grad=True), p_drop=p_attn, keepmask=lse[1])
+                wg, wt = ar.qkv_wgrad(i), ar.wt[('qkv', i)]
+                ops.gemm_wgrad_pair(dq_c, h_c, wg[:d], dAO, ctx_c, ar.g(a + 'out_lin.weight'))
+                ops.gemm_wgrad(dkv, h_in, wg[d:])
+                dh_ = ops.gemm_nt(dkv, wt[:, d:], L.EPI_NONE)
+                dh_q = ops.gemm_nt(dq_c, wt[:, :d], L.EPI_RES, aux=dpre1)
+                ops.scatter_add_rows(dh_q, rows_c.idx, dh_, rows_c.n, d)
+                del dq_c, dkv, dh_q, q_c, kv, h_c, dctx, dAO, dpre1, dx1
+                ar.touch_layer(i)
+                if hook is not None:
+                    hook.layer_done(i, last)
+                continue
             if compact:
                 ops.gemm_wgrad(dAO, ctx_c, ar.g(a + 'out_lin.weight'))
                 dctx = ops.place_rows(dctx, rows_c.inv, M, 0)
diff --git a/m3p_amd/lib.py b/m3p_amd/lib.py
--- a/m3p_amd/lib.py
+++ b/m3p_amd/lib.py
@@ -47,6 +47,8 @@
     'm3p_layernorm_bwd_rows': (_i, [_p, _p, _p, _p, _p, _p, _p, _p, _p, _p, _p, _p, _i, _i, _u32, _u32, _f, _p, _p]),
     'm3p_attn_fwd': (_i, [_p, _p, _p, _p, _p, _i, _i, _i, _i, _u32, _u32, _f, _p]),
     'm3p_attn_bwd': (_i, [_p, _p, _p, _p, _p, _p, _p, _p, _i, _i, _i, _i, _f, _u32, _u32, _f, _p]),
+    'm3p_attn_fwd_listed': (_i, [_p, _p, _i, _p, _p, _p, _i, _p, _p, _p, _i, _i, _i, _i, _u32, _u32, _f, _p]),
+    'm3p_attn_bwd_listed': (_i, [_p, _p, _i, _p, _p, _p, _i, _p, _p, _p, _p, _p, _p, _i, _p, _i, _i, _i, _i, _f, _u32, _f, _p]),
     'm3p_attn_query_fwd': (_i, [_p, _i, _p, C.c_longlong, _i, _p, _p, _i, _i, _i, _i, _i, _i, _i, _p]),
     'm3p_attn_query_owner_fwd': (_i, [_p, _i, _p, C.c_longlong, _i, _p, _p, _i, _i, _i, _i, _i, _i, _i, _p, _i, _i, _p]),
     'm3p_vocab_select_max_k': (_i, []),
diff --git a/m3p_amd/ops.py b/m3p_amd/ops.py
--- a/m3p_amd/ops.py
+++ b/m3p_amd/ops.py
@@ -296,6 +296,48 @@
     return dqkv
 
 
+def attn_listed_eligible(S, dh):
+    return dh == 64 and (S + 15) // 16 == 11 and S % 2 == 0
+
+
+def attn_fwd_listed(q, kv, keylen, q_off, q_ent, B, S, H, dh, seed=0, p_drop=0.0):
+    _chk_bf16(q, kv)
+    n, d = q.shape
+    assert d == H * dh and q.is_contiguous() and kv.shape[0] == B * S and kv.shape[1] >= 2 * d and kv.stride(1) == 1
+    assert keylen.dtype == torch.int32 and q_off.dtype == torch.int32 and q_ent.dtype == torch.int32
+    assert q_off.is_cuda and q_ent.is_cuda and q_off.is_contiguous() and q_ent.is_contiguous()
+    assert q_off.numel() == B + 1 and q_ent.numel() == n
+    ctx = torch.empty((n, d), dtype=BF16, device=q.device)
+    lse = torch.empty((H, n), dtype=torch.float32, device=q.device)
+    mask = None
+    if p_drop > 0:
+        nt = (S + 15) // 16
+        mask = torch.empty((B * H, nt, nt, 4), dtype=torch.int64, device=q.device)
+    rc = L.load().m3p_attn_fwd_listed(q.data_ptr(), kv.data_ptr(), kv.stride(0), keylen.data_ptr(), q_off.data_ptr(),
+                                      q_ent.data_ptr(), n, ctx.data_ptr(), lse.data_ptr(), L.ptr(mask), B, S, H, dh, seed,
+                                      L.thresh24(p_drop), 1.0 / (1.0 - p_drop) if p_drop > 0 else 1.0, L.stream())
+    L.check(rc, 'm3p_attn_fwd_listed')
+    return ctx, lse, mask
+
+
+def attn_bwd_listed(q, kv, keylen, q_off, q_ent, ctx, dctx, lse, B, S, H, dh, dbias_qkv=None, p_drop=0.0, keepmask=None):
+    _chk_bf16(q, kv, ctx, dctx)
+    n, d = q.shape
+    assert q.is_contiguous() and ctx.is_contiguous() and dctx.is_contiguous() and ctx.shape == (n, d) and dctx.shape == (n, d)
+    assert kv.shape[0] == B * S and kv.shape[1] >= 2 * d and kv.stride(1) == 1 and lse.shape == (H, n) and lse.is_contiguous()
+    assert q_off.numel() == B + 1 and q_ent.numel() == n and q_off.dtype == torch.int32 and q_ent.dtype == torch.int32
+    assert p_drop == 0 or keepmask is not None, 'attention backward with dropout needs the keep words of the forward pass'
+    dq = torch.empty((n, d), dtype=BF16, device=q.device)
+    dkv = torch.empty((B * S, 2 * d), dtype=BF16, device=q.device)
+    rc = L.load().m3p_attn_bwd_listed(q.data_ptr(), kv.data_ptr(), kv.stride(0), keylen.data_ptr(), q_off.data_ptr(),
+                                      q_ent.data_ptr(), n, ctx.data_ptr(), dctx.data_ptr(), lse.data_ptr(), L.ptr(keepmask),
+                                      dq.data_ptr(), dkv.data_ptr(), dkv.stride(0), L.ptr(dbias_qkv), B, S, H, dh,
+                                      1.0 / (dh ** 0.5), L.thresh24(p_drop), 1.0 / (1.0 - p_drop) if p_drop > 0 else 1.0,
+                                      L.stream())
+    L.check(rc, 'm3p_attn_bwd_listed')
+    return dq, dkv
+
+
 def attn_query_fwd(q, kv, klen, B, Tq, H, dh, Lk, causal=False, pos0=0, owner=None):
     _chk_bf16(q, kv)
     assert q.stride(1) == 1 and kv.dim() == 3 and kv.stride(2) == 1 and kv.shape[1] >= Lk
```

Result: no change. 8113 sequences/s, median of 6 (+0.5%).
